# tpatten/squirrel_motion_planner

Hardware: AMD Instinct MI355X
Metric: collision-checked samples/sec + time-to-first-feasible-path, 8-DoF, 5 cm octomap (higher is better)
Workload: dtype f64

## Files before the change

### include/smp_gpu.h

```cpp
#ifndef SMP_GPU_H
#define SMP_GPU_H

#include <stddef.h>
#include <stdint.h>

#ifdef __cplusplus
extern "C" {
#endif

enum {
  SMP_OK = 0,
  SMP_ERR_ARG = -1,
  SMP_ERR_START_INVALID = -2,
  SMP_ERR_GOAL_INVALID = -3,
  SMP_ERR_NO_SOLUTION = -4,
  SMP_ERR_HIP = -5,
  SMP_ERR_PARSE = -6,
  SMP_ERR_CAPACITY = -7,
  SMP_ERR_NO_DEVICE = -8
};

enum { SMP_BUDGET_ITERATIONS = 0, SMP_BUDGET_SECONDS = 1, SMP_BUDGET_SAMPLES = 2 };

typedef struct smp_robot smp_robot;
typedef struct smp_scene smp_scene;
typedef struct smp_planner smp_planner;

typedef struct smp_scene_opts {
  double resolution;
  double z_offset;
  int insert_floor;
  double floor_center[2];
  double floor_distance;
} smp_scene_opts;

typedef struct smp_params {
  double near_threshold;
  double step_factor;
  int num_traj_segments;
  int max_near_nodes;
  double path_optimality_threshold;
  int tree_optimization;
  int informed_sampling;
  int64_t node_capacity;
  int helpers;
  int scout;
} smp_params;

typedef struct smp_query {
  double start[8];
  double goal[8];
  double env_x[2];
  double env_y[2];
  int check_self;
  int check_map;
  int budget_kind;
  double budget;
  uint64_t seed;
  uint32_t query_id;
} smp_query;

typedef struct smp_stats {
  int64_t iterations;
  int64_t first_solution_iter;
  int64_t last_solution_iter;
  int64_t configs_checked;
  int64_t configs_valid;
  double time_first_solution;
  double time_total;
  double cost_best[3];
  double cost_theoretical[3];
  int64_t nodes_start, nodes_goal, edges_start, edges_goal, rewires_start, rewires_goal;
  int32_t connected_tree_is_start;
  int32_t conn_node_b, conn_node_a;
  int64_t nn_nodes_scanned;
  int64_t near_nodes_scanned;
  int64_t samples_precomputed;
  double phase_seconds[32];
  int64_t scout_nn_hits;
  int64_t scout_near_hits;
  int64_t scout_edge_hits;
  int64_t scout_edge_misses;
  double scout_wait_seconds;
  double scout_phase_seconds[32];
  int32_t helpers;
  int32_t scout;
  double time_first_solution_host;
  int64_t scout_conn_row_hits;
  int64_t scout_conn_batch_hits;
  int64_t scout_conn_ov_hits;
} smp_stats;

typedef struct smp_result {
  int status;
  int64_t n_waypoints;
  double* waypoints;
  smp_stats stats;
  int64_t n_cost_rows;
  double* cost_rows;
} smp_result;

void smp_params_default(smp_params* p);
void smp_scene_opts_default(smp_scene_opts* o);

int smp_robot_create_json(const char* model_json, smp_robot** out);
int smp_robot_create_urdf(const char* urdf_xml, const char* srdf_xml, const char* spheres_json, smp_robot** out);
void smp_robot_destroy(smp_robot* r);
int smp_robot_num_links(const smp_robot* r);
const char* smp_robot_link_name(const smp_robot* r, int i);
int smp_robot_self_rounds(const smp_robot* r, int32_t info[8], uint16_t* sp_ab, double* sp_rr2, uint16_t* pp_ps,
                          int32_t* partner, double* rr2, uint32_t* prim_mask);

typedef struct smp_attach {
  const char* link;
  const char* name;
  int n_spheres;
  const double* centres;
  const double* radii;
  const char* const* touch_links; int n_touch;
} smp_attach;
int smp_robot_attach(const smp_robot* base, const smp_attach* a, smp_robot** out);
int smp_cover_box(const double half[3], const double pose[12], double tol, int max_spheres,
                  double* centres, double* radii, int* n);
int smp_cover_cylinder(double radius, double half_length, const double pose[12], double tol, int max_spheres,
                       double* centres, double* radii, int* n);

int smp_scene_from_keys(const uint16_t* keys_xyz, int64_t n, const smp_scene_opts* opts, smp_scene** out);
int smp_scene_from_bt(const uint8_t* data, size_t size, const smp_scene_opts* opts, smp_scene** out);
int smp_scene_from_ot(const uint8_t* data, size_t size, const smp_scene_opts* opts, smp_scene** out);
int smp_scene_from_octomap_msg(const char* id, double resolution, int binary, const uint8_t* data, size_t size,
                               const smp_scene_opts* opts, smp_scene** out);
int smp_scene_from_grid(const uint64_t* bits, const uint16_t* d2, const int dims[3], const double origin[3],
                        double resolution, smp_scene** out);
void smp_scene_destroy(smp_scene* s);
int smp_scene_info(const smp_scene* s, int dims[3], double origin[3], double* resolution,
                   int64_t* n_occupied, double bbox_min[3], double bbox_max[3]);
int smp_scene_export(const smp_scene* s, uint64_t* bits, uint16_t* d2);

int smp_planner_create(int device, const smp_robot* robot, const smp_params* params, smp_planner** out);
void smp_planner_destroy(smp_planner* p);
int smp_planner_set_scene(smp_planner* p, const smp_scene* s);
typedef struct smp_scene_build {
  int dims[3];
  double origin[3];
  double resolution;
  int64_t n_occupied;
  double bbox_min[3], bbox_max[3];
  double kernel_ms;
  double total_ms;
} smp_scene_build;
int smp_planner_set_scene_keys(smp_planner* p, const uint16_t* keys_xyz, int64_t n, const smp_scene_opts* opts,
                               smp_scene_build* info);
int smp_planner_set_scene_bt(smp_planner* p, const uint8_t* data, size_t size, const smp_scene_opts* opts,
                             smp_scene_build* info);
int smp_planner_set_scene_ot(smp_planner* p, const uint8_t* data, size_t size, const smp_scene_opts* opts,
                             smp_scene_build* info);
int smp_planner_set_scene_octomap_msg(smp_planner* p, const char* id, double resolution, int binary,
                                      const uint8_t* data, size_t size, const smp_scene_opts* opts,
                                      smp_scene_build* info);
typedef struct smp_carve {
  double q[8];
  double pad;
  const char* const* links; int n_links;
} smp_carve;
typedef struct smp_carve_info { int64_t n_carved; double kernel_ms, total_ms; } smp_carve_info;
int smp_planner_set_carve(smp_planner* p, const smp_carve* c);
int smp_planner_last_carve(const smp_planner* p, smp_carve_info* info);
int smp_carve_keys(smp_planner* p, const uint16_t* keys_xyz, int64_t n, const smp_scene_opts* opts,
                   const smp_carve* c, uint8_t* carved, smp_carve_info* info);
int smp_planner_set_params(smp_planner* p, const smp_params* params);
int smp_planner_get_params(const smp_planner* p, smp_params* params);
int smp_set_disabled_map_links(smp_planner* p, const char* const* link_names, int n);
int smp_planner_set_robot(smp_planner* p, const smp_robot* r);
// ... 183 lines not shown
```

### squirrel_motion_planner_amd/_lib.py

```python
import ctypes
import os

HERE = os.path.dirname(os.path.abspath(__file__))
LIB_PATH = os.environ.get("SMP_LIB") or os.path.join(HERE, "lib", "libsmp_gpu.so")
MODEL_JSON = os.path.join(HERE, "data", "robotino_model.json")
SPHERES_JSON = os.path.join(HERE, "data", "robotino_spheres.json")

SMP_OK = 0
SMP_ERR_ARG = -1
SMP_ERR_START_INVALID = -2
SMP_ERR_GOAL_INVALID = -3
SMP_ERR_NO_SOLUTION = -4
SMP_ERR_HIP = -5
SMP_ERR_PARSE = -6
SMP_ERR_CAPACITY = -7
SMP_ERR_NO_DEVICE = -8

BUDGET_ITERATIONS = 0
BUDGET_SECONDS = 1
BUDGET_SAMPLES = 2

_d = ctypes.c_double
_i = ctypes.c_int
_i64 = ctypes.c_int64
_p = ctypes.c_void_p
_pd = ctypes.POINTER(ctypes.c_double)


class SceneOpts(ctypes.Structure):
    _fields_ = [("resolution", _d), ("z_offset", _d), ("insert_floor", _i), ("floor_center", _d * 2),
                ("floor_distance", _d)]


class Params(ctypes.Structure):
    _fields_ = [("near_threshold", _d), ("step_factor", _d), ("num_traj_segments", _i), ("max_near_nodes", _i),
                ("path_optimality_threshold", _d), ("tree_optimization", _i), ("informed_sampling", _i),
                ("node_capacity", _i64), ("helpers", _i), ("scout", _i)]


class Query(ctypes.Structure):
    _fields_ = [("start", _d * 8), ("goal", _d * 8), ("env_x", _d * 2), ("env_y", _d * 2), ("check_self", _i),
                ("check_map", _i), ("budget_kind", _i), ("budget", _d), ("seed", ctypes.c_uint64),
                ("query_id", ctypes.c_uint32)]


class Stats(ctypes.Structure):
    _fields_ = [("iterations", _i64), ("first_solution_iter", _i64), ("last_solution_iter", _i64),
                ("configs_checked", _i64), ("configs_valid", _i64), ("time_first_solution", _d), ("time_total", _d),
                ("cost_best", _d * 3), ("cost_theoretical", _d * 3), ("nodes_start", _i64), ("nodes_goal", _i64),
                ("edges_start", _i64), ("edges_goal", _i64), ("rewires_start", _i64), ("rewires_goal", _i64),
                ("connected_tree_is_start", ctypes.c_int32), ("conn_node_b", ctypes.c_int32),
                ("conn_node_a", ctypes.c_int32), ("nn_nodes_scanned", _i64), ("near_nodes_scanned", _i64),
                ("samples_precomputed", _i64), ("phase_seconds", _d * 32), ("scout_nn_hits", _i64),
                ("scout_near_hits", _i64), ("scout_edge_hits", _i64), ("scout_edge_misses", _i64),
                ("scout_wait_seconds", _d), ("scout_phase_seconds", _d * 32), ("helpers", ctypes.c_int32),
                ("scout", ctypes.c_int32), ("time_first_solution_host", _d), ("scout_conn_row_hits", _i64),
                ("scout_conn_batch_hits", _i64), ("scout_conn_ov_hits", _i64)]


class Result(ctypes.Structure):
    _fields_ = [("status", _i), ("n_waypoints", _i64), ("waypoints", _pd), ("stats", Stats), ("n_cost_rows", _i64),
                ("cost_rows", _pd)]


class IkRequest(ctypes.Structure):
    _fields_ = [("ee_pose", _d * 6), ("deviation", (_d * 2) * 6), ("q_init", _d * 8), ("max_iter", _i)]


class IkResult(ctypes.Structure):
    _fields_ = [("reached", _i), ("iterations", _i), ("fallback_iterations", _i), ("q", _d * 8), ("error", _d * 6),
                ("manipulability", _d)]


class GoalSearch(ctypes.Structure):
    _fields_ = [("n_candidates", _i), ("n_reached", _i), ("chosen", _i), ("downward", _i), ("kernel_ms", _d)]


class SceneDevice(ctypes.Structure):
    _fields_ = [("dims", _i * 3), ("origin", _d * 3), ("resolution", _d), ("n_bricks", _i64), ("n_cells", _i64),
                ("n_prim", _i), ("has_d2b", _i), ("bricks", _p), ("d2", _p), ("d2b", _p), ("slab", _p)]


class SceneBuild(ctypes.Structure):
    _fields_ = [("dims", _i * 3), ("origin", _d * 3), ("resolution", _d), ("n_occupied", _i64), ("bbox_min", _d * 3),
                ("bbox_max", _d * 3), ("kernel_ms", _d), ("total_ms", _d)]


class Attach(ctypes.Structure):
    _fields_ = [("link", ctypes.c_char_p), ("name", ctypes.c_char_p), ("n_spheres", _i), ("centres", _pd),
                ("radii", _pd), ("touch_links", ctypes.POINTER(ctypes.c_char_p)), ("n_touch", _i)]


class Carve(ctypes.Structure):
    _fields_ = [("q", _d * 8), ("pad", _d), ("links", ctypes.POINTER(ctypes.c_char_p)), ("n_links", _i)]


class CarveInfo(ctypes.Structure):
    _fields_ = [("n_carved", _i64), ("kernel_ms", _d), ("total_ms", _d)]


class ShortcutInfo(ctypes.Structure):
    _fields_ = [("n_edges", _i64), ("n_valid", _i64), ("configs_checked", _i64), ("cost_in", _d), ("cost_out", _d),
                ("first_blocked", _i64), ("kernel_ms", _d), ("total_ms", _d)]


class Detour(ctypes.Structure):
    _fields_ = [("v", _d * 8), ("M1", ctypes.c_int32), ("M2", ctypes.c_int32), ("free", ctypes.c_int32),
                ("pad", ctypes.c_int32)]


class RepairOpts(ctypes.Structure):
    _fields_ = [("samples", _i), ("rounds", _i), ("seed", ctypes.c_uint64)]


class RepairInfo(ctypes.Structure):
    _fields_ = [("n_blocked_edges", _i64), ("n_gaps", _i64), ("n_repaired", _i64), ("n_items", _i64), ("n_free", _i64),
                ("rounds_used", ctypes.c_int32), ("cost_in", _d), ("cost_out", _d), ("first_blocked", _i64),
                ("kernel_ms", _d), ("total_ms", _d)]


class Margin(ctypes.Structure):
    _fields_ = [("map", _d), ("self", _d)]


class Clearance(ctypes.Structure):
    _fields_ = [("map", _d), ("self", _d), ("map_link", ctypes.c_int32), ("self_a", ctypes.c_int32),
                ("self_b", ctypes.c_int32), ("pad", ctypes.c_int32)]


class EdgeClearance(ctypes.Structure):
    _fields_ = [("map", _d), ("self", _d), ("map_point", ctypes.c_int32), ("self_point", ctypes.c_int32),
                ("map_link", ctypes.c_int32), ("self_a", ctypes.c_int32), ("self_b", ctypes.c_int32),
                ("n_points", ctypes.c_int32)]


class ClearanceInfo(ctypes.Structure):
    _fields_ = [("n_points", _i64), ("kernel_ms", _d), ("total_ms", _d)]


class BaseLattice(ctypes.Structure):
# ... 171 lines not shown
```

### squirrel_motion_planner_amd/csrc/smp_api_plan.cpp

```cpp
#include <hip/hip_runtime.h>

#include <algorithm>
#include <array>
#include <chrono>
#include <cmath>
#include <cstdio>
#include <cstdlib>
#include <cstring>
#include <thread>
#include <vector>

#include "smp_kernels.h"
#include "smp_planner.h"
#include "smp_provision.h"

using namespace smp;

static_assert(PROV_MAX_SCOUTS == MAX_SCOUTS && PROV_SCAN_P == SCAN_P && PROV_SCAN_PNEAR == SCAN_PNEAR,
              "smp_provision.h restates smp_plan.h");

static int resident_slots(smp_planner* p) {
  if (p->slots_cache > 0) return std::max(1, p->slots_cache / std::max(1, p->slot_share));
  int occ_plan = 0;
  if (hipOccupancyMaxActiveBlocksPerMultiprocessor(&occ_plan, reinterpret_cast<const void*>(&plan_kernel), BLOCK, 0) !=
// ... 435 lines not shown
    if (k.bounds) {
      int dbg[8];
      if (smp_debug_bounds(dbg) == 0 && dbg[0])
        std::fprintf(stderr, "[smp] bounds: %s:%d id %d block %d tree %d limit %d (launch %lld)\n", site_file(dbg[0]),
                     site_line(dbg[0]), dbg[1], dbg[2], dbg[3], dbg[4], (long long)c.launches);
    }
    float ms = 0;
    HIPCHK(hipEventElapsedTime(&ms, p->ev0, p->ev1));
    c.total_ms += ms;
    if (k.debug) {
      JobBoard jbh;
      const int i0 = act[0];
      if (nh > 0) HIPCHK(hipMemcpy(&jbh, c.qdev[i0].jb, sizeof(JobBoard), hipMemcpyDeviceToHost));
      std::fprintf(stderr, "[smp] launch %lld queries %d grid %d chunk %d: %.3f ms phase %d status %d iter %lld checked %lld"
                   " board stop %d job %u tile0 %llx\n", (long long)c.launches, na, na * (1 + nh), chunk, ms, S[i0].phase,
                   S[i0].status, S[i0].iter, S[i0].checked, nh ? jbh.stop : -1, nh ? (unsigned)(jbh.pay[0] >> 32) : 0u,
                   nh ? jbh.res[0] : 0ull);
    }
    std::vector<int> still;
    int solved_before = 0, solved_now = 0;
    for (int i : act) solved_before += sol_seen[i];
    for (int i : act)
      if (!(S[i].phase == 2 || S[i].status != 0)) still.push_back(i);
    for (int i : act) { sol_seen[i] = S[i].have_sol ? 1 : 0; solved_now += sol_seen[i]; }
    const bool shrank = still.size() < act.size();
    act.swap(still);
    if (act.empty()) break;
    if (shrank || (ns > c.prov.ns_base && solved_now != solved_before)) {
      if (k.rebalance) provision_queries(c, act);
      if (int st = upload_active(c)) return st;
    }
    if (chunk < 4096) chunk *= 2;
  }
  hstamp(c, "launch loop done");
#ifdef SMP_RING_CHECK
  smp_ringchk_dump();
#endif
  return SMP_OK;
}

static int plan_assemble(PlanCall& c, smp_result* out, std::vector<char>& done) {
  smp_planner* p = c.p;
  const int nq = c.nq;
  QState* S = c.S;
  HIPCHK(hipMemcpyAsync(p->d_qdev.p, c.qdev.data(), nq * sizeof(QueryDev), hipMemcpyHostToDevice, p->stream));
  p->last_plan_ms = c.total_ms;
  p->last_plan_launches = c.launches;

  hipLaunchKernelGGL(path_kernel, dim3(nq), dim3(64), 0, p->stream, p->d_qdev.p, p->d_counts.p);
  HIPCHK(hipGetLastError());
  std::vector<int> counts(2 * nq);
  HIPCHK(hipMemcpyAsync(counts.data(), p->d_counts.p, 2 * nq * sizeof(int), hipMemcpyDeviceToHost, p->stream));
  HIPCHK(hipStreamSynchronize(p->stream));
  int rc = SMP_OK;
  for (int i = 0; i < nq; ++i) {
    QState& s = S[i];
    smp_result& r = out[i];
    r.status = s.status != 0 ? s.status : (s.have_sol ? SMP_OK : SMP_ERR_NO_SOLUTION);
    smp_stats& st = r.stats;
    st.iterations = s.iter;
    st.first_solution_iter = s.first_iter;
    st.last_solution_iter = s.last_iter;
    st.configs_checked = s.checked;
    st.configs_valid = s.valid;
    st.time_first_solution = s.have_sol && s.t_first >= s.t0 ? (double)(s.t_first - s.t0) / p->wall_rate_hz : -1.0;
    st.time_total = s.t_end >= s.t0 ? (double)(s.t_end - s.t0) / p->wall_rate_hz : 0.0;
    st.time_first_solution_host = s.have_sol ? c.host_ttff[i] : -1.0;
    for (int k = 0; k < 3; ++k) { st.cost_best[k] = s.cbest[k]; st.cost_theoretical[k] = s.h0[k]; }
    st.nodes_start = s.n[0]; st.nodes_goal = s.n[1];
    st.edges_start = s.edges[0]; st.edges_goal = s.edges[1];
    st.rewires_start = s.rewires[0]; st.rewires_goal = s.rewires[1];
    st.connected_tree_is_start = s.conn_start;
    st.conn_node_b = s.nB.id; st.conn_node_a = s.nA.id;
    st.nn_nodes_scanned = s.nn_nodes;
    st.near_nodes_scanned = s.near_nodes;
    st.samples_precomputed = s.smp_hits;
    st.scout_nn_hits = s.sc_nn;
    st.scout_near_hits = s.sc_near;
    st.scout_edge_hits = s.sc_edge_hit;
    st.scout_edge_misses = s.sc_edge_miss;
    st.scout_conn_row_hits = s.sc_conn_row;
    st.scout_conn_batch_hits = s.sc_conn_batch;
    st.scout_conn_ov_hits = (int64_t)c.scout_conn_ov[i];
    st.scout_wait_seconds = (double)s.sc_wait / p->wall_rate_hz;
    for (int k = 0; k < 32; ++k) {
      const bool count = k == 8 || k == 11 || (k >= 20 && k < 28) || k == 30;
      st.scout_phase_seconds[k] = count ? (double)c.scout_prof[i][k] : (double)c.scout_prof[i][k] / p->wall_rate_hz;
    }
    st.helpers = c.nh_first;
    st.scout = c.ns_first;
    for (int k = 0; k < 32; ++k)
      st.phase_seconds[k] = (k == 8 || k == 11 || k >= 20) ? (double)s.prof[k] : (double)s.prof[k] / p->wall_rate_hz;
    if (i == 0) { p->last_n[0] = s.n[0]; p->last_n[1] = s.n[1]; }
    r.n_cost_rows = s.n_rows;
    if (s.n_rows > 0) {
      r.cost_rows = (double*)malloc(sizeof(double) * 5 * s.n_rows);
      HIPCHK(hipMemcpy(r.cost_rows, p->qb[i].rows.p, sizeof(double) * 5 * s.n_rows, hipMemcpyDeviceToHost));
      for (int64_t k = 0; k < s.n_rows; ++k) r.cost_rows[k * 5 + 1] /= p->wall_rate_hz;
    }
    if (r.status != SMP_OK) { done[i] = 1; continue; }
    const int n_sp = counts[2 * i], n_gp = counts[2 * i + 1];
    const int np = p->params.num_traj_segments;
    std::vector<double> pe((size_t)(n_sp + n_gp) * 2 * NJ);
    if (n_sp + n_gp > 0) {
      HIPCHK(p->d_path_edges.reserve(pe.size()));
      const int nthr = (int)pe.size();
      hipLaunchKernelGGL(path_edges_kernel, dim3((nthr + 255) / 256), dim3(256), 0, p->stream, p->d_qdev.p, i, n_sp,
                         n_gp, p->d_path_edges.p);
      HIPCHK(hipGetLastError());
      HIPCHK(hipMemcpyAsync(pe.data(), p->d_path_edges.p, pe.size() * sizeof(double), hipMemcpyDeviceToHost, p->stream));
      HIPCHK(hipStreamSynchronize(p->stream));
    }
    std::vector<double> wp;
    for (int k = 0; k < n_sp + n_gp; ++k) {
      const double* a = &pe[(size_t)k * 2 * NJ];
      const double* b = a + NJ;
      double stp[NJ];
      for (int j = 0; j < NJ; ++j) stp[j] = (b[j] - a[j]) / double(np);
      if (k < n_sp) {
        for (int inc = 0; inc < np; ++inc)
          for (int j = 0; j < NJ; ++j) wp.push_back(a[j] + inc * stp[j]);
      } else {
        for (int inc = np; inc > 0; --inc)
          for (int j = 0; j < NJ; ++j) wp.push_back(a[j] + inc * stp[j]);
        if (k == n_sp + n_gp - 1)
          for (int j = 0; j < NJ; ++j) wp.push_back(a[j] + 0 * stp[j]);
      }
    }
    r.n_waypoints = (int64_t)(wp.size() / NJ);
    if (!wp.empty()) {
      r.waypoints = (double*)malloc(sizeof(double) * wp.size());
      std::memcpy(r.waypoints, wp.data(), sizeof(double) * wp.size());
    }
    done[i] = 1;
  }
  for (int i = 0; i < nq; ++i) if (out[i].status != SMP_OK && rc == SMP_OK) rc = out[i].status;
  hstamp(c, "results assembled");
  return rc;
}

static int plan_batch_impl(smp_planner* p, const smp_query* qs, int nq, smp_result* out, std::vector<char>& done) {
  PlanCall c;
  c.t_entry = std::chrono::steady_clock::now();
  c.p = p;
  c.qs = qs;
  c.nq = nq;
  c.k = read_plan_knobs(p->params.helpers, nq);
  if (int st = plan_prepare(c)) return st;
  if (int st = plan_launch_loop(c)) return st;
  return plan_assemble(c, out, done);
}

extern "C" int smp_plan_batch(smp_planner* p, const smp_query* qs, int nq, smp_result* out) {
  if (!p || !qs || nq <= 0 || !out) return SMP_ERR_ARG;
  for (int i = 0; i < nq; ++i) std::memset(&out[i], 0, sizeof(smp_result));
  if (int b_ = busy_check(p)) {
    for (int i = 0; i < nq; ++i) out[i].status = b_;
    return b_;
  }
  std::vector<char> done(nq, 0);
  const int rc = plan_batch_impl(p, qs, nq, out, done);
  if (rc == SMP_ERR_HIP) (void)hipGetLastError();
  for (int i = 0; i < nq; ++i) {
    if (done[i]) continue;
    smp_result_free(&out[i]);
    out[i].status = rc != SMP_OK ? rc : SMP_ERR_HIP;
// ... 73 lines not shown
```

### squirrel_motion_planner_amd/csrc/smp_kernels.hip

```cpp
#include <hip/hip_runtime.h>

#include <vector>

#include "smp_collide.h"
#include "smp_kernels.h"
#include "smp_math.h"
#include "smp_plan.h"
#include "smp_types.h"

extern "C" __device__ __attribute__((const)) unsigned long long __ockl_wfred_min_u64(unsigned long long);
extern "C" __device__ __attribute__((const)) unsigned long long __ockl_wfred_max_u64(unsigned long long);

namespace smp {

constexpr int CHECK_CT = 32;

__shared__ RobotDev g_rb;
__shared__ MapCfg g_mc;
__shared__ WideStash g_wk;

template <int CT>
__global__ void __launch_bounds__(BLOCK) check_kernel_t(const RobotDev* __restrict__ rb, SceneDev sc,
                                                        const MapCfg* __restrict__ mc, const double* __restrict__ q,
                                                        long long n, int self, int map, uint8_t* __restrict__ valid,
// ... 271 lines not shown
static_assert(sizeof(ViaNode) == 8 * (3 * NJ + 3 + 1), "ViaNode as 8-byte words: q, c, e_start, e_target, {id, parent}");
static_assert(VIA_B * VIA_WORDS <= BLOCK, "one ViaNode word per thread");
struct PlanLds {
  QState S;
  union {
    struct {
      TileLds<PLAN_CT> T;
      double tq[PLAN_CT][NJ];
    } tile;
    JobLds job;
    double seg[MAXE][MAX_PTS][3];
    ViaLds via;
    SmpLds smp;
    SamplerLds smpl;
  } u;
  union {
    struct {
      struct {
        unsigned long long wlk[BLOCK / 64][MAX_NEAR], whk[BLOCK / 64][MAX_NEAR];
        int wli[BLOCK / 64][MAX_NEAR], whi[BLOCK / 64][MAX_NEAR];
        int wtot[BLOCK / 64];
      } nr;
      struct {
        alignas(16) unsigned hist[NEAR_BINS];
        unsigned long long ck[2][NEAR_BUF];
        int ci[2][NEAR_BUF];
        unsigned long long wmin[BLOCK / 64], wmax[BLOCK / 64];
        int wtot[BLOCK / 64];
        int cnt[2], blo, bhi, fast;
      } nh;
    };
    struct {
      ScanLds s;
      MergeLds m;
    } sc;
  };
  double eg_start[MAXE][NJ], eg_target[MAXE][NJ], eg_step[MAXE][NJ], eg_end[MAXE][NJ];
  double eg_base[MAXE][3], eg_cost[MAXE][3];
  double eg_acc[MAXE][3];
  int eg_first[MAXE], eg_need[MAXE], eg_near[MAXE], eg_ptr[MAXE];
  int eg_par[MAXE];
  int conn_need0;
  int rw_par[MAXE], rw_next;
  double rw_cost[MAXE][3];
  int tile_e[PLAN_CT], tile_i[PLAN_CT], tile_n;
  int count_slot;
  int job_seq;
  int in_job;
  int go_end;
  int smp_ver, smp_have_sol, smp_hit;
  int smp_pub;
  int spec, spec_nn;
  long long spec_cnt;
  double smp_cbest[3];
  int nk;
  unsigned long long near_blo, near_bhi;
  int lo_i[MAX_NEAR], hi_i[MAX_NEAR];
  double lo_c[MAX_NEAR], hi_c[MAX_NEAR];
  int n_lo, n_hi;
  NodeRef nn, xn, xc, cur, g;
  double xr[NJ], ext[NJ], ox[NJ];
  double en_start[NJ], en_target[NJ];
  int ext_nn, ext_bp, flag, found, nn_id, cnt;
  int reached;
  int n_via, nn_t, tree_expand;
  NodeRef sel;
  double sel_start[NJ], sel_target[NJ];
  double csp[3], best_nv;
  double sol[3];
  double wd[BLOCK / 64];
  unsigned long long wk[BLOCK / 64];
  int wi[BLOCK / 64];
  long long wcount[BLOCK / 64];
  ScoutRec sr;
  PreRec prer;
  int prer_ok;
#ifdef SMP_TRACE
  int trole;
  unsigned tn;
  long long tit;
  int tbar;
#endif
  int sp_on, sp_stage, sp_go[2];
  double fnn_d;
  int fnn_id;
#ifdef SMP_SCAN_PROF
  unsigned long long spc_t;
#endif
  int sc_same[MAX_SCOUTS];
  unsigned sc_seen, sc_dead;
  int asked[SCOUT_SLOTS];
  int asked_conn[SCOUT_SLOTS];
  int asked_pre[SCOUT_SLOTS];
  int two_scouts;
  unsigned sc_mod;
  unsigned rw_at0;
  int n_at0;
  int sc_t, sc_rerun;
  int sc_stale_f;
  int ov_local, conn_ov;
  unsigned conn_ov_n;
#ifdef SMP_CONN_PROF
  unsigned cprof[12];
#endif
  double sc_hq[MAXE][NJ], sc_hc[MAXE];
  int sc_hp[MAXE];
  int rb_go[2];
  long long sc_k;
  int eg_hit[MAXE];
  int eg_rec[MAXE];
  int rec_grp;
  int rec_all, ev_job;
  double pc_q[2][PATCH_K][NJ];
};

__shared__ PlanLds g_L;
static_assert(sizeof(ViaLds) <= sizeof(g_L.u.seg), "a via chain's batch lies within the union's edge rows");

struct Ctx {
  SceneDev sc;
  QueryDev Q;
};

}
#include "smp_plan_prof.h"
namespace smp {

__device__ __forceinline__ int lane_id() { return threadIdx.x & 63; }
__device__ __forceinline__ int uni(int v) { return __builtin_amdgcn_readfirstlane(v); }
__device__ __forceinline__ int wave_id() { return threadIdx.x >> 6; }
typedef const double __attribute__((address_space(1)))* gcdptr;
__device__ __forceinline__ gcdptr uni_gptr(const double* p) {
  const unsigned long long v = reinterpret_cast<unsigned long long>(p);
  const unsigned lo = __builtin_amdgcn_readfirstlane((int)(unsigned)v);
  const unsigned hi = __builtin_amdgcn_readfirstlane((int)(unsigned)(v >> 32));
  return (gcdptr)(((unsigned long long)hi << 32) | lo);
}

__device__ __forceinline__ gcdptr uni_g(gcdptr p) {
  const unsigned long long v = reinterpret_cast<unsigned long long>(p);
  const unsigned lo = __builtin_amdgcn_readfirstlane((int)(unsigned)v);
  const unsigned hi = __builtin_amdgcn_readfirstlane((int)(unsigned)(v >> 32));
  return (gcdptr)(((unsigned long long)hi << 32) | lo);
}
__device__ __forceinline__ void tree_cols(gcdptr tq, int cap, gcdptr* c) {
#pragma unroll
  for (int j = 0; j < NJ; ++j) c[j] = uni_g(tq + (size_t)j * (unsigned)cap);
}
__device__ __forceinline__ bool wave_group_live(int first, int end) {
  return __builtin_amdgcn_readfirstlane((int)(first < end)) != 0;
}
__device__ __forceinline__ double ld_col(gcdptr col, unsigned i) {
  return *(gcdptr)((const char __attribute__((address_space(1)))*)col + i * 8u);
}
typedef const float __attribute__((address_space(1)))* gcfptr;
__device__ __forceinline__ float ld_col(gcfptr col, unsigned i) {
  return *(gcfptr)((const char __attribute__((address_space(1)))*)col + i * 4u);
}
template <int K, int NPT, typename P, typename T>
__device__ __forceinline__ void load_round_k(T (*a)[NJ], const P* cols, int b0, int i1, const T* fill) {
#pragma unroll
  for (int u = 0; u < NPT; ++u) {
    if (u < K) {
      const unsigned ii = (unsigned)min(b0 + u * BLOCK, i1 - 1);
#pragma unroll
      for (int j = 0; j < NJ; ++j) a[u][j] = ld_col(cols[j], ii);
    } else {
#pragma unroll
      for (int j = 0; j < NJ; ++j) a[u][j] = fill[j];
    }
  }
}
template <int NPT, typename P, typename T>
__device__ __forceinline__ void load_round(T (*a)[NJ], const P* cols, int b0, int i1, const T* fill) {
  static_assert(NPT == 8, "rounds of 8 nodes per thread");
  const int first = b0 - lane_id();
  const int nl = uni(min(NPT, (i1 - first + BLOCK - 1) / BLOCK));
  if (nl > 4) load_round_k<8, NPT>(a, cols, b0, i1, fill);
  else if (nl > 2) load_round_k<4, NPT>(a, cols, b0, i1, fill);
  else if (nl > 1) load_round_k<2, NPT>(a, cols, b0, i1, fill);
  else load_round_k<1, NPT>(a, cols, b0, i1, fill);
}

__device__ __forceinline__ void st_tree(double* p, double v) { *p = v; }
__device__ __forceinline__ void st_tree(int* p, int v) { *p = v; }
__device__ __forceinline__ void st_tree(float* p, float v) { *p = v; }
__device__ __forceinline__ void st_coord(const TreeDev& T, int cap, int j, int i, double v) {
  st_tree(&T.q[(size_t)j * cap + i], v);
  st_tree(&T.qf[(size_t)j * cap + i], (float)v);
}
__device__ __forceinline__ int xcc_id() { return __builtin_amdgcn_s_getreg((3 << 11) | 20); }
__device__ __forceinline__ bool same8(const double* a, const double* b) {
  bool s = true;
#pragma unroll
  for (int j = 0; j < NJ; ++j) s &= __double_as_longlong(a[j]) == __double_as_longlong(b[j]);
  return s;
}

#define load_node(C, t, id, o) load_node_at(C, t, id, o, SMP_SITE)
__device__ __forceinline__ void load_node_at(const Ctx& C, int t, int id, NodeRef* o, int site) {
  const TreeDev& T = C.Q.tr[t];
  const int cap = g_L.S.cap;
  BCHK(id, cap, site, t);
  (void)site;
  for (int j = 0; j < NJ; ++j) o->q[j] = T.q[(size_t)j * cap + id];
  for (int k = 0; k < 3; ++k) o->c[k] = T.cost[(size_t)k * cap + id];
  o->id = id;
  o->parent = T.parent[id];
}

__device__ void insert_node(const Ctx& C, int t, const double* e_start, const double* e_target, const NodeRef& x) {
  QState& S = g_L.S;
  int i = S.n[t];
  if (i >= S.cap || x.id != i) { S.status = -7; S.phase = 2; return; }
  const TreeDev& T = C.Q.tr[t];
  int cap = S.cap;
  for (int j = 0; j < NJ; ++j) {
    st_coord(T, cap, j, i, x.q[j]);
    T.e_start[(size_t)j * cap + i] = e_start[j];
    T.e_target[(size_t)j * cap + i] = e_target[j];
    g_L.pc_q[t][i & (PATCH_K - 1)][j] = x.q[j];
  }
  for (int k = 0; k < 3; ++k) st_tree(&T.cost[(size_t)k * cap + i], x.c[k]);
  st_tree(&T.parent[i], x.parent);
  T.first_child[i] = -1;
  int p = x.parent;
  int f = T.first_child[p];
  T.next_sib[i] = f;
  T.prev_sib[i] = -1;
  if (f >= 0) T.prev_sib[f] = i;
  T.first_child[p] = i;
  S.n[t] = i + 1;
  S.edges[t]++;
}

__device__ bool spec_stage(const Ctx& C, int s, unsigned long long wait = 0);
__device__ __forceinline__ int scan_parts(const Ctx& C, int near, int nodes) {
  int P = min(min(C.Q.nworkers, SCAN_P), near ? min(min(C.Q.scan_pnear, SCAN_PNEAR), max(8, nodes >> C.Q.scan_nshift)) : C.Q.scan_pnn);
  if (g_L.in_job) P = min(P, max(C.Q.nworkers - g_L.u.job.ntiles, 8));
  return uni(P);
}
__device__ __forceinline__ bool scan_split(const Ctx& C, int nodes) {
  return uni(C.Q.jb != nullptr && C.Q.scan_min > 0 && nodes >= C.Q.scan_min && C.Q.nworkers >= 8 && !g_L.ov_local);
}
__device__ int nearest_dist(const Ctx& C, int t, const double* q, int i0, int n, double* d_out);
__device__ void near_set_dist(const Ctx& C, int t, const double* q, int excl, bool nn);
constexpr int LOCAL_F32_MIN = 2048;
struct ScanLds;
__device__ __forceinline__ void slice_nn_body32(gcdptr tq, const float* tqf, int cap, int i0, int i1, const double* q,
                                                ScanLds& X);
__device__ __forceinline__ int nearest_scan(const Ctx& C, int t, const double* q, int i_begin, double* d_out) {
  TR();
  if (scan_split(C, uni(g_L.S.n[t]) - i_begin)) {
    int id;
    [[clang::always_inline]] id = nearest_dist(C, t, q, i_begin, uni(g_L.S.n[t]), d_out);
    return id;
  }
  const gcdptr tq = uni_gptr(C.Q.tr[t].q);
  const int n = uni(g_L.S.n[t]), cap = uni(g_L.S.cap);
  if (n - i_begin >= LOCAL_F32_MIN) {
    slice_nn_body32(tq, C.Q.tr[t].qf, cap, i_begin, n, q, g_L.sc.s);
    *d_out = __longlong_as_double((long long)g_L.sc.s.wk[0]);
    const int id = g_L.sc.s.wi[0];
    __syncthreads();
    return id;
  }
  gcdptr tqc[NJ];
  tree_cols(tq, cap, tqc);
  double qq[NJ];
  for (int j = 0; j < NJ; ++j) qq[j] = q[j];
  double best = 10000.0, best_s = 1e300;
  int bid = 0x7fffffff;
  constexpr int NPT = 8;
  for (int i0 = i_begin + threadIdx.x; i0 < n; i0 += NPT * BLOCK) {
    double a[NPT][NJ];
    load_round<NPT>(a, tqc, i0, n, qq);
    double s[NPT];
#pragma unroll
    for (int u = 0; u < NPT; ++u) s[u] = 0.0;
#pragma unroll
    for (int j = 0; j < NJ; ++j) {
#pragma unroll
      for (int u = 0; u < NPT; ++u) {
        const double d = qq[j] - a[u][j];
        s[u] += d * d;
      }
    }
#pragma unroll
    for (int u = 0; u < NPT; ++u) {
      const int i = i0 + u * BLOCK;
      if (i < n && s[u] < best_s) {
        const double dist = sqrt(s[u]);
        if (dist < best) { best = dist; bid = i; best_s = s[u]; }
      }
    }
  }
  TR();
  const unsigned long long key = (unsigned long long)__double_as_longlong(best);
  const unsigned long long wk = __ockl_wfred_min_u64(key);
  const int wi = __ockl_wfred_min_i32(key == wk ? bid : 0x7fffffff);
  if (lane_id() == 0) { g_L.wk[wave_id()] = wk; g_L.wi[wave_id()] = wi; }
  __syncthreads();
  unsigned long long bk = g_L.wk[0];
  int bi = g_L.wi[0];
#pragma unroll
  for (int w = 1; w < BLOCK / 64; ++w) {
    const unsigned long long k = g_L.wk[w];
    const int i = g_L.wi[w];
    if (k < bk || (k == bk && i < bi)) { bk = k; bi = i; }
  }
  __syncthreads();
  *d_out = __longlong_as_double((long long)bk);
  TR();
  return bi;
}

__device__ int patch_scan(int t, const double* q, int i0, int n, double* d_out) {
  if (threadIdx.x < 64) {
    const int i = i0 + (int)threadIdx.x;
// ... 1416 lines not shown
    }
    const unsigned long long lb = __ballot(live);
    if (lane == 0) J.tskip = lb == 0;
  }
  __syncthreads();
  return uni(J.tskip) != 0;
}

struct DirectJob {
  unsigned hdr;
  int ne;
};
__device__ __forceinline__ unsigned job_tile_mask(const Ctx& C, const WideConst& K, JobLds& J, int t,
                                                  unsigned long long* prof = nullptr, int seq = -1,
                                                  const DirectJob* direct = nullptr, bool sync_after = true) {
  int ct, nc, self, map;
  bool sk = false;
  if (direct) {
    const unsigned hdr = direct->hdr;
    const int ne = direct->ne;
    const int np1 = (int)((hdr >> 8) & 255);
    ct = 1 << ((hdr >> 21) & 3);
    const int base = t * ct;
    nc = min(ct, ne * np1 - base);
    self = (int)((hdr >> 16) & 1);
    map = (int)((hdr >> 17) & 1);
    const int c = (int)(threadIdx.x >> 6) / (NWAVE / ct), j = threadIdx.x & 63;
    if (c < nc && j < NJ) {
      const int sl = base + c, k = sl / np1, i = sl - k * np1, wi = 1 + 32 * k + 2 * j;
      const double qs = __hiloint2double((int)J.words[wi + 1], (int)J.words[wi]);
      const double qd = __hiloint2double((int)J.words[wi + 2 * NJ + 1], (int)J.words[wi + 2 * NJ]);
      J.tq[c][j] = qs + i * qd;
    }
    wave_sync();
  } else {
    ct = uni(J.ct);
    const int base = t * ct;
    nc = min(ct, uni(J.nslots) - base);
    self = J.self;
    map = J.map;
    sk = seq >= 0 && uni(J.skip) && t >= uni(C.Q.nworkers);
    if (sk && job_tile_skip(C, J, t, seq)) return 0u;
    if (threadIdx.x < nc * NJ) {
      const int c = threadIdx.x / NJ, j = threadIdx.x - c * NJ;
      const int sl = base + c, k = sl / J.np1, i = sl - k * J.np1;
      J.tq[c][j] = J.start[k][j] + i * J.step[k][j];
    }
    if (threadIdx.x < TILE_CT_MAX) J.T.coll[threadIdx.x] = 0;
    __syncthreads();
  }
  const TileOrder order{J.tgrp, J.tord, J.first, false};
  collide_wide((&g_rb), K, ct, nc, J.tq, self, map, J.T, sk ? &order : nullptr, prof);
  unsigned m = 0;
  for (int c = 0; c < nc; ++c) m |= (J.T.coll[c] ? 1u : 0u) << c;
  if (sync_after) __syncthreads();
  return m;
}

__device__ __noinline__ unsigned job_tile_mask_out(const Ctx& C, JobLds& J, int t, int seq) {
  const WideConst K = wide_const_load(g_wk, C.sc);
  return job_tile_mask(C, K, J, t, nullptr, seq);
}

enum { OV_NONE = 0, OV_NEAR_EXPAND = 1, OV_NN = 2, OV_NEAR_XN = 3 };
__device__ void overlap_work(const Ctx& C, int ov, int t);
__device__ void conn_window(const Ctx& C, int t);
__device__ __forceinline__ bool take_spec(int ov) {
  const bool hit = uni(g_L.spec) == ov;
  __syncthreads();
  if (hit && threadIdx.x == 0) {
    (ov == OV_NN ? g_L.S.nn_nodes : g_L.S.near_nodes) += g_L.spec_cnt;
    g_L.spec = OV_NONE;
  }
  __syncthreads();
  return hit;
}

enum { EARLY_NONE = 0, EARLY_EXPAND = 1, EARLY_CHOOSE = 2, EARLY_REWIRE = 3 };
constexpr int EDGE_EARLY_W = (int)(offsetof(ScoutEdge, first) / 8);
static_assert(EDGE_EARLY_W == 2 * NJ + 3, "ScoutEdge: s, g, acc, then {first, pad}");
__device__ __forceinline__ int sc_stale_now(const ScoutBoard* sb) {
  return (long long)ld_agent(&sb->cur) > g_L.sc_k || ld_agent(&sb->stop);
}
__device__ __forceinline__ void sc_early_send(const Ctx& C, int early, int epar, int E, bool read_stale) {
  if (early == EARLY_NONE) return;
  ScoutBoard* sb = C.Q.scb;
  ScoutRec* rec = &sb->rec[epar];
  if (read_stale && threadIdx.x == 0) g_L.sc_stale_f = sc_stale_now(sb);
  const int g0 = early == EARLY_EXPAND ? 0 : early == EARLY_CHOOSE ? SCOUT_CHOOSE0 : SCOUT_REWIRE0;
  for (int i = threadIdx.x; i < E * EDGE_EARLY_W; i += BLOCK) {
    const int e = i / EDGE_EARLY_W, k = i - e * EDGE_EARLY_W;
    const double v = k < NJ ? g_L.eg_start[e][k] : k < 2 * NJ ? g_L.eg_target[e][k - NJ] : g_L.eg_acc[e][k - 2 * NJ];
    st_agent(reinterpret_cast<unsigned long long*>(&rec->e[g0 + e]) + k, (unsigned long long)__double_as_longlong(v));
  }
  if (early == EARLY_EXPAND) {
    constexpr int XW = (int)(sizeof(ScoutExpand) / 8);
    static_assert(XW == 3 * NJ + 3 + 1 && offsetof(ScoutExpand, ok) == (XW - 1) * 8, "ScoutExpand: ext, step, end, acc, {ok, pad}");
    const int k = (int)threadIdx.x - 64;
    if (k >= 0 && k < XW) {
      unsigned long long w;
      if (k == XW - 1) w = *reinterpret_cast<const unsigned long long*>(&g_L.sr.ex.ok);
      else w = (unsigned long long)__double_as_longlong(k < NJ ? g_L.eg_target[0][k] : k < 2 * NJ ? g_L.eg_step[0][k - NJ] :
                                                        k < 3 * NJ ? g_L.eg_end[0][k - 2 * NJ] : g_L.eg_acc[0][k - 3 * NJ]);
      st_agent(reinterpret_cast<unsigned long long*>(&rec->ex) + k, w);
    }
  } else {
    const int k = (int)threadIdx.x - (BLOCK - 64);
    if (k >= 0 && k < 2) st_agent(reinterpret_cast<unsigned long long*>(&rec->n_choose) + k,
                                  reinterpret_cast<const unsigned long long*>(&g_L.sr.n_choose)[k]);
  }
}
__device__ __forceinline__ void sc_first_send(const Ctx& C, int early, int epar, int E) {
  const int g0 = early == EARLY_EXPAND ? 0 : early == EARLY_CHOOSE ? SCOUT_CHOOSE0 : SCOUT_REWIRE0;
  if ((int)threadIdx.x < E) {
    const int e = threadIdx.x;
    const int first = g_L.eg_need[e] ? g_L.eg_first[e] : -1;
    st_agent(reinterpret_cast<unsigned long long*>(&C.Q.scb->rec[epar].e[g0 + e]) + EDGE_EARLY_W,
             (unsigned long long)(unsigned)first);
  }
}

__device__ __forceinline__ void job_header(const Ctx& C, bool need, bool sfv) {
  auto& J = g_L.u.job;
  const int e = threadIdx.x;
  const int np1 = g_L.S.n_pts + 1;
  const int W = max(1, C.Q.nworkers);
  const unsigned long long m = __ballot(need);
  const int k = __popcll(m & ((1ull << e) - 1));
  if (need) J.emap[k] = e;
  if (e == 0) {
    const int ne = __popcll(m);
    J.E = ne;
    J.np1 = np1;
    J.nslots = ne * np1;
    J.ct = job_tile_ct(ne * np1, W, C.Q.tile_ct);
    J.ntiles = (ne * np1 + J.ct - 1) / J.ct;
    J.self = g_L.S.self; J.map = g_L.S.map;
    J.seq = ++g_L.job_seq;
    J.skip = J.ntiles > W;
    J.sfv = J.skip && sfv;
  }
}
__device__ __forceinline__ void edge_validity_job(const Ctx& C, int E, int pslot, int ov, int ovt, int early = 0,
                                                  int epar = 0, bool conn_b = false) {
  JobBoard* jb = C.Q.jb;
  auto& J = g_L.u.job;
  const int np1 = g_L.S.n_pts + 1;
  const int W = max(1, C.Q.nworkers);
  const int ne = uni(J.E), nt = uni(J.ntiles), seq = uni(J.seq), ct = uni(J.ct);
  const unsigned long long tj0 = threadIdx.x == 0 ? wall_clock64() : 0;
  for (int i = threadIdx.x; i < 1 + 32 * ne; i += BLOCK) {
    unsigned w;
    if (i == 0) {
      w = (unsigned)ne | (unsigned)np1 << 8 | (unsigned)(J.self != 0) << 16 | (unsigned)(J.map != 0) << 17 |
          (unsigned)J.skip << 19 | (unsigned)J.sfv << 20 | (unsigned)__builtin_ctz((unsigned)J.ct) << 21;
    } else {
      const int m = i - 1, k = m >> 5, r = m & 31, j = (r & 15) >> 1, e = J.emap[k];
      const unsigned long long bits = (unsigned long long)__double_as_longlong(r < 16 ? g_L.eg_start[e][j] : g_L.eg_step[e][j]);
      w = (r & 1) ? (unsigned)(bits >> 32) : (unsigned)bits;
    }
    st_agent(&jb->pay[i], granule(seq, w));
  }
  for (int it = threadIdx.x; it < ne * NJ; it += BLOCK) {
    const int k = it / NJ, j = it - k * NJ, e = J.emap[k];
    J.start[k][j] = g_L.eg_start[e][j];
    J.step[k][j] = g_L.eg_step[e][j];
  }
  for (int t = threadIdx.x; t < nt; t += BLOCK) J.rdone[t] = 0;
  if (threadIdx.x < ne) J.first[threadIdx.x] = np1;
  JOBPROF_PUBLISHED(jb);
  PROF_BEGIN();
  if (threadIdx.x == 0) { g_L.S.prof[P_TFK] += _pt - tj0; g_L.S.prof[P_TTEST]++; }
  TR();
  if (threadIdx.x == 0) g_L.in_job = 1;
  sc_early_send(C, early, epar, E, false);
  __syncthreads();
  if (conn_b) conn_window(C, ovt);
  else overlap_work(C, ov, ovt);
  if (threadIdx.x == 0) g_L.in_job = 0;
  TR();
  const bool skip = uni(J.skip) != 0;
  for (int t = W - 1; t < nt; t += W) {
    const unsigned m = job_tile_mask_out(C, J, t, skip ? seq : -1);
    if (threadIdx.x == 0) {
      J.rmask[t] = m;
      J.rdone[t] = 1;
      if (skip) st_agent(&jb->res[t], granule(seq, m));
    }
  }
  __syncthreads();
  const unsigned long long tj1 = threadIdx.x == 0 ? wall_clock64() : 0;
  if (threadIdx.x == 0) g_L.S.prof[P_TCHAIN] += tj1 - _pt;
  unsigned long long t_prog = tj1, t_wait = tj1;
  int last_left = 1 << 30;
  for (int k = 0;; k ^= 1) {
    if (threadIdx.x < 64) {
      int left = 0;
      unsigned long long cur_v = 0;
      int stop_v = 0;
      if (early != EARLY_NONE && threadIdx.x == 0) { cur_v = ld_agent(&C.Q.scb->cur); stop_v = ld_agent(&C.Q.scb->stop); }
      for (int t = threadIdx.x; t < nt; t += 64) {
// ... 447 lines not shown
      }
      if (go > 0 && threadIdx.x < TILE_CT_MAX) J.T.coll[threadIdx.x] = 0;
      if (threadIdx.x == 0) {
        if (go == 0 && (ld_agent(&jb->stop) || wall_clock64() - t_last > 200000000ull)) go = -1;
        J.go[k] = go;
        J.seq = go == -3 ? (int)stag : (int)tag0;
      }
    }
    __syncthreads();
    const int go = uni(J.go[k]);
    if (go == -1) break;
    if (go == 0) {
      __builtin_amdgcn_s_sleep(SMP_HELPER_SLEEP);
      continue;
    }
    const int seq = uni(J.seq);
    if (go == -3) {
      scan_helper(C, J, w, seq);
      last_scan = seq;
      t_last = wall_clock64();
      continue;
    }
    const unsigned hdr = J.words[0];
    const int ne = min((int)(hdr & 255), MAXE), nw = 1 + 32 * ne;
    if (go == -2) {
      int bad = 0;
      for (int i = PU * 64 + threadIdx.x; i < nw; i += BLOCK) {
        const unsigned long long v = ld_agent(&jb->pay[i]);
        if ((int)(v >> 32) != seq) bad = 1;
        J.words[i] = (unsigned)v;
      }
      if (threadIdx.x == 0) J.left = 0;
      __syncthreads();
      if (bad) J.left = 1;
      __syncthreads();
      if (uni(J.left)) continue;
    }
    auto decode = [&]() {
      for (int it = threadIdx.x; it < ne * 2 * NJ; it += BLOCK) {
        const int kk = it / (2 * NJ), r = it - kk * 2 * NJ;
        const int wi = 1 + 32 * kk + 2 * r;
        const double d = __hiloint2double((int)J.words[wi + 1], (int)J.words[wi]);
        if (r < NJ) J.start[kk][r] = d; else J.step[kk][r - NJ] = d;
      }
      if (threadIdx.x == 0) {
        J.E = ne;
        J.np1 = (int)((hdr >> 8) & 255);
        J.self = (hdr >> 16) & 1;
        J.map = (hdr >> 17) & 1;
        J.skip = (hdr >> 19) & 1;
        J.sfv = (hdr >> 20) & 1;
        J.nslots = ne * J.np1;
        J.ct = 1 << ((hdr >> 21) & 3);
        J.ntiles = (J.nslots + J.ct - 1) / J.ct;
      }
      if (hdr & (1u << 19))
        for (int t = threadIdx.x; t < JOB_TILES; t += BLOCK) J.rdone[t] = 0;
    };
    JOBPROF_TILE_CLOCKS(J, tp);
    const int nt = (ne * (int)((hdr >> 8) & 255) + (1 << ((hdr >> 21) & 3)) - 1) >> ((hdr >> 21) & 3);
    const bool direct = go > 0;
    last = seq;
    JOBPROF_PICKUP(jb, w, nt);
    if (w - 1 >= nt) __syncthreads();
    bool decoded = false;
    const DirectJob dj{hdr, ne};
    for (int t = w - 1; t < nt; t += W) {
      const bool dt = direct && t == w - 1;
      if (!dt && !decoded) {
        decode();
        __syncthreads();
        decoded = true;
      }
      const unsigned m = job_tile_mask(C, K, J, t, tp, seq, dt ? &dj : nullptr, false);
      if (threadIdx.x == 0) st_agent(&jb->res[t], granule(seq, m));
      __syncthreads();
      JOBPROF_TILE_DONE(jb);
    }
    JOBPROF_TILES_OUT(jb, J, w, nt);
    t_last = wall_clock64();
  }
}

__device__ __forceinline__ void sc_copy_out(ScoutBoard* sb, int par, const void* p, int nbytes) {
  const size_t off = (const char*)p - (const char*)&g_L.sr;
  const unsigned long long* src = (const unsigned long long*)p;
  unsigned long long* dst = (unsigned long long*)((char*)&sb->rec[par] + off);
  for (int w = threadIdx.x; w < nbytes / 8; w += BLOCK) st_agent(&dst[w], src[w]);
}
__device__ __forceinline__ void sc_copy_in(const ScoutBoard* sb, int par, void* p, int nbytes) {
  const size_t off = (const char*)p - (const char*)&g_L.sr;
  unsigned long long* dst = (unsigned long long*)p;
  const unsigned long long* src = (const unsigned long long*)((const char*)&sb->rec[par] + off);
  for (int w = threadIdx.x; w < nbytes / 8; w += BLOCK) dst[w] = ld_agent(&src[w]);
}
static_assert(sizeof(ScoutNN) % 8 == 0 && sizeof(ScoutNear) % 8 == 0 && sizeof(ScoutEdge) % 8 == 0 &&
              sizeof(ScoutExpand) % 8 == 0 && offsetof(ScoutRec, ex) % 8 == 0 && offsetof(ScoutRec, nr) % 8 == 0 &&
              sizeof(ScoutConnect) % 8 == 0 && offsetof(ScoutRec, cn) % 8 == 0 && sizeof(ScoutConn) % 8 == 0 &&
              sizeof(ScoutPre) % 8 == 0 && offsetof(ScoutRec, pre) % 8 == 0 && sizeof(ViaNode) % 8 == 0 &&
              offsetof(ScoutRec, cc) % 8 == 0 && offsetof(ScoutRec, n_choose) % 8 == 0 && offsetof(ScoutRec, e) % 8 == 0,
              "scout record sections are 8-byte words");

constexpr unsigned long long SCOUT_WAIT = 6000;
#ifndef SMP_CONN_WAIT
#define SMP_CONN_WAIT 2000
#endif

__device__ void spec_copy(const ScoutBoard* sb, int par, int have, int st);
__device__ bool spec_stage(const Ctx& C, int s, unsigned long long wait) {
  if (!uni(g_L.sp_on)) return false;
  if (wait == 0) wait = SCOUT_WAIT;
  const int have = uni(g_L.sp_stage);
  if (have >= s) return true;
  const ScoutBoard* sb = C.Q.scbs[uni(g_L.asked[g_L.S.iter & (SCOUT_SLOTS - 1)]) - 1];
  const int par = (int)(g_L.S.iter & (SCOUT_SLOTS - 1));
  const unsigned tag = (unsigned)(g_L.S.iter + 1);
  const unsigned long long t0 = threadIdx.x == 0 ? wall_clock64() : 0;
  TR();
  int got;
  for (int k = 0;; k ^= 1) {
    if (threadIdx.x == 0) {
      const unsigned long long v = ld_agent(&sb->stage[par]);
      const unsigned lo = (unsigned)v;
      const bool cur = ((lo >> 8) & 0xfffu) == (g_L.rw_at0 & 0xfffu);
      int go = 0;
      if ((unsigned)(v >> 32) != tag) go = -1;
      else if (cur && (int)(lo & 0xffu) >= s) go = 1 + (int)(lo & 0xffu);
      else if (wall_clock64() - t0 > wait) go = -1;
      g_L.sp_go[k] = go;
    }
    __syncthreads();
    got = uni(g_L.sp_go[k]);
    if (got != 0) break;
    __builtin_amdgcn_s_sleep(1);
  }
  if (threadIdx.x == 0) g_L.S.sc_wait += wall_clock64() - t0;
  WAIT_CLOCK(s, t0);
  TR();
  if (got < 0) {
    if (threadIdx.x == 0) g_L.sp_on = 0;
    __syncthreads();
    return false;
  }
  spec_copy(sb, par, have, got - 1);
  TR();
  return true;
}

__device__ void spec_copy(const ScoutBoard* sb, int par, int have, int st) {
  ScoutRec& R = g_L.sr;
  const bool opt_now = uni(g_L.S.tree_opt && g_L.S.have_sol) != 0;
  int off[8], nw[8], ns = 0;
  auto add = [&](const void* p, int nbytes) {
    off[ns] = (int)((const char*)p - (const char*)&R) / 8;
    nw[ns] = nbytes / 8;
    ++ns;
  };
  if (have < SC_NN && st >= SC_NN) add(&R.nn, sizeof(ScoutNN));
  if (have < SC_EXPAND && st >= SC_EXPAND) { add(&R.e[0], sizeof(ScoutEdge)); add(&R.ex, sizeof(ScoutExpand)); }
  if (have < SC_NEAR && st >= SC_NEAR) add(&R.nr, sizeof(ScoutNear));
  if ((have < SC_CHOOSE && st >= SC_CHOOSE) || (have < SC_DONE && st >= SC_DONE)) add(&R.n_choose, 4 * sizeof(int));
  if (opt_now && have < SC_CHOOSE && st >= SC_CHOOSE) add(&R.e[SCOUT_CHOOSE0], MAX_NEAR * sizeof(ScoutEdge));
  if (opt_now && have < SC_DONE && st >= SC_DONE) add(&R.e[SCOUT_REWIRE0], MAX_NEAR * sizeof(ScoutEdge));
  if (!opt_now && have < SC_DONE && st >= SC_DONE) { add(&R.cn, sizeof(ScoutConnect)); add(&R.pre, sizeof(ScoutPre)); }
  if (have < SC_CONN && st >= SC_CONN) add(&R.cc, sizeof(ScoutConn));
  int total = 0;
  for (int i = 0; i < ns; ++i) total += nw[i];
  const unsigned long long* src = reinterpret_cast<const unsigned long long*>(&sb->rec[par]);
  unsigned long long* dst = reinterpret_cast<unsigned long long*>(&R);
  constexpr int U = 4;
  static_assert(sizeof(ScoutRec) / 8 <= U * BLOCK, "one round per record copy");
  int idx[U];
  unsigned long long v[U];
#pragma unroll
  for (int u = 0; u < U; ++u) {
    const int w = (int)threadIdx.x + u * BLOCK;
    idx[u] = -1;
    if (w < total) {
      int rem = w, i = 0;
      while (rem >= nw[i]) { rem -= nw[i]; ++i; }
      idx[u] = off[i] + rem;
      v[u] = ld_agent(&src[idx[u]]);
    }
  }
#pragma unroll
  for (int u = 0; u < U; ++u)
    if (idx[u] >= 0) dst[idx[u]] = v[u];
  __syncthreads();
  if (threadIdx.x == 0) g_L.sp_stage = st;
  __syncthreads();
}

__device__ void scout_ask(const Ctx& C, long long k, int tree, bool pre, bool& fenced, int x_snap = -1) {
  const QState& S = g_L.S;
  const int ns = C.Q.nscouts;
  int which = 1 + (int)(pre ? (unsigned)k % (unsigned)ns : (ns >= 2 ? (unsigned)(k & 1) : 0u));
  if ((g_L.sc_dead >> (which - 1)) & 1u) {
    if (!pre) return;
    int w = -1;
    for (int d = 1; d < ns && w < 0; ++d) {
      const int c = (int)((unsigned)(k + d) % (unsigned)ns);
      if (!((g_L.sc_dead >> c) & 1u)) w = c;
    }
    if (w < 0) return;
    for (int x = 0; x < SCOUT_SLOTS; ++x)
      if (g_L.asked[x] == 1 + w) return;
    which = 1 + w;
  }
  ScoutBoard* sb = C.Q.scbs[which - 1];
  int& same = g_L.sc_same[which - 1];
  if (same < 0) {
    const int x = ld_agent(&sb->xcc);
    if (x > 0) same = (x - 1) == xcc_id() ? 1 : 0;
  }
  if (same != 1 && !fenced) {
    __builtin_amdgcn_fence(__ATOMIC_RELEASE, "agent");
    drain();
    fenced = true;
  }
  const unsigned tag = (unsigned)(k + 1);
  const unsigned w0 = (unsigned)(x_snap >= 0 ? x_snap : S.n[tree]) | (unsigned)tree << 28 | (unsigned)(!pre) << 29;
  st_agent(&sb->req[2], granule(tag, (unsigned)S.n[1 - tree]));
  st_agent(&sb->req[1], granule(tag, ((unsigned)g_L.smp_ver & 0xfffffu) | ((unsigned)S.rewires[tree] & 0xfffu) << 20));
  st_agent(&sb->req[0], granule(tag, w0));
  g_L.asked[k & (SCOUT_SLOTS - 1)] = which;
  g_L.asked_conn[k & (SCOUT_SLOTS - 1)] = !pre && ns >= 2;
  g_L.asked_pre[k & (SCOUT_SLOTS - 1)] = pre;
}

__device__ void scout_ask_early(const Ctx& C, int stage_j) {
  const QState& S = g_L.S;
  if (!C.Q.early_ask || C.Q.nscouts < 2 || !(S.tree_opt && S.have_sol) || stage_j < SC_DONE) return;
  const long long k = S.iter + 2;
  if (g_L.asked[k & (SCOUT_SLOTS - 1)]) return;
  const int w = (int)(k & 1);
  if (g_L.sc_same[w] != 1 || ((g_L.sc_dead >> w) & 1u)) return;
  bool fenced = true;
  scout_ask(C, k, S.A, false, fenced, g_L.n_at0);
}

__device__ void scout_slots() {
  const QState& S = g_L.S;
  const long long j = S.iter;
  g_L.rw_at0 = (unsigned)S.rewires[S.A];
  g_L.n_at0 = S.n[S.A];
  g_L.asked[(j - 1) & (SCOUT_SLOTS - 1)] = 0;
  g_L.asked_conn[(j - 1) & (SCOUT_SLOTS - 1)] = 0;
  g_L.sp_on = g_L.asked[j & (SCOUT_SLOTS - 1)] != 0 &&
              !(g_L.asked_pre[j & (SCOUT_SLOTS - 1)] && S.have_sol && j >= S.first_iter + 3);
  g_L.sp_stage = -1;
}
__device__ __forceinline__ void scout_cur_lanes(const Ctx& C) {
  const QState& S = g_L.S;
  const long long j = S.iter;
  const int s = (int)lane_id();
  if (s >= C.Q.nscouts) return;
  const bool pre = !(S.tree_opt && S.have_sol);
  const int nsc = pre ? C.Q.nscouts : min(C.Q.nscouts, 2);
  ScoutBoard* sb = C.Q.scbs[s];
  if (!pre && j == S.first_iter + 3 && s >= 2) st_agent(&sb->stop, 1);
  if (s >= nsc) return;
  st_agent(&sb->cur, (unsigned long long)j);
  if (pre && S.n[0] < (1 << 20) && S.n[1] < (1 << 20) && g_L.sc_same[s] == 1)
    st_agent(&sb->cur_sz, ((unsigned long long)(j & 0xffffff) << 40) | ((unsigned long long)S.n[0] << 20) |
                              (unsigned long long)S.n[1]);
}
__device__ void scout_asks(const Ctx& C, int t) {
  const QState& S = g_L.S;
  const long long j = S.iter;
  const bool pre = !(S.tree_opt && S.have_sol);
  bool fenced = false;
  for (int ahead = 1; ahead <= (pre ? C.Q.nscouts : 1); ++ahead) {
    const long long k = j + ahead;
// ... 650 lines not shown
      for (int i = 0; i < 2; ++i) {
        double s = 0.0;
        for (int k = 0; k < 2; ++k) s += (S.Cpr[i * 2 + k] * lp[k]) * bp[k];
        rp[i] = s + S.ctr_pr[i];
      }
      {
        int cr = 0, cp = 0;
#pragma unroll
        for (int j = 0; j < NJ; ++j) {
          const bool rv = rb->rev[j] != 0;
          double v = 0.0;
#pragma unroll
          for (int i = 0; i < 6; ++i) v = rv && cr == i ? rr[i] : v;
#pragma unroll
          for (int i = 0; i < 2; ++i) v = !rv && cp == i ? rp[i] : v;
          r[j] = v;
          cr += rv ? 1 : 0;
          cp += rv ? 0 : 1;
        }
      }
      bool above = 0.0 <= ee_z(rb, r);
      bool inside = (r[0] < S.env_x[1] && r[0] > S.env_x[0] && r[1] < S.env_y[1] && r[1] > S.env_y[0]) || env0;
      unsigned long long m = __ballot(above && inside && lane < SE_OUT);
      const int w = m ? __ffsll((long long)m) - 1 : -1;
      if (lane == w) for (int j = 0; j < NJ; ++j) out[j] = r[j];
      if (lane == 0) W.win = w;
    }
    __syncthreads();
    if (uni(W.win) >= 0) return 0;
  }
}

__device__ __forceinline__ int sample_conf(const QState& S, uint32_t it, SmpLds& W, double* out) {
  if (uni(S.informed && S.have_sol)) return sample_ellipse(S, it, W, out);
  return sample_uniform(S, it, W, out);
}

__device__ void sample_version(const Ctx& C) {
  QState& S = g_L.S;
  g_L.smp_pub = 0;
  if (!C.Q.sampler) return;
  const bool changed = g_L.smp_ver == 0 || g_L.smp_have_sol != S.have_sol || g_L.smp_cbest[0] != S.cbest[0] ||
                       g_L.smp_cbest[1] != S.cbest[1] || g_L.smp_cbest[2] != S.cbest[2];
  if (changed) {
    g_L.smp_have_sol = S.have_sol;
    for (int k = 0; k < 3; ++k) g_L.smp_cbest[k] = S.cbest[k];
    ++g_L.smp_ver;
    g_L.smp_pub = 1;
  }
}
__device__ void sample_publish(const Ctx& C, bool before_read = false) {
  if (!C.Q.sampler) return;
  const QState& S = g_L.S;
  JobBoard* jb = C.Q.jb;
  if (g_L.smp_pub) {
    st_agent(&jb->s_have_sol, g_L.smp_have_sol);
    for (int k = 0; k < 3; ++k) st_agent(&jb->s_cbest[k], (unsigned long long)__double_as_longlong(g_L.smp_cbest[k]));
    drain();
    st_agent(&jb->s_ver, g_L.smp_ver);
  }
  st_agent(reinterpret_cast<unsigned long long*>(&jb->s_iter), (unsigned long long)(S.iter - (before_read ? 1 : 0)));
}

__device__ __forceinline__ bool pre_read_round(const ScoutBoard* sb, int par, unsigned tag) {
  const int g = (int)threadIdx.x - 64;
  if (g < 0 || g >= PRE_GRANULES) return true;
  const unsigned long long v = ld_agent(&sb->pre_g[par][g]);
  reinterpret_cast<unsigned*>(&g_L.prer)[g] = (unsigned)v;
  return (unsigned)(v >> 32) == tag;
}

__device__ __forceinline__ void sample_read(const Ctx& C) {
  TR();
  QState& S = g_L.S;
  const uint32_t it = (uint32_t)S.iter;
  const bool pre = uni(g_L.sp_on && g_L.sp_stage < 0) != 0;
  const int sw = uni(g_L.asked[S.iter & (SCOUT_SLOTS - 1)]);
  const ScoutBoard* sb = sw > 0 ? C.Q.scbs[sw - 1] : nullptr;
  const int par = (int)(S.iter & (SCOUT_SLOTS - 1));
  const bool prerec = pre && !uni(S.have_sol);
  bool pre_ok = true;
  if (prerec) pre_ok = pre_read_round(sb, par, (unsigned)(S.iter + 1));
  if (threadIdx.x == 64) {
    int st = -1;
    if (pre && !prerec) {
      const unsigned long long v = ld_agent(&sb->stage[par]);
      const unsigned lo = (unsigned)v;
      if ((unsigned)(v >> 32) == (unsigned)(S.iter + 1) && ((lo >> 8) & 0xfffu) == (g_L.rw_at0 & 0xfffu))
        st = (int)(lo & 0xffu);
    }
    g_L.sp_go[0] = st;
  }
  if (C.Q.sampler && threadIdx.x < 64) {
    JobBoard* jb = C.Q.jb;
    const unsigned want = ring_tag(it, (unsigned)__builtin_amdgcn_readfirstlane(g_L.smp_ver));
    unsigned long long v = 0;
    if (threadIdx.x < RING_G) v = ld_agent(&jb->ring[it % SMP_RING].g[threadIdx.x]);
    const int pk = (int)threadIdx.x - 2 * NJ;
    const bool ok = threadIdx.x >= RING_G ||
                    ((unsigned)(v >> 32) == want && (pk < 0 || (unsigned)v == ring_param(pk, S.have_sol, S.cbest)));
    const unsigned hi = (unsigned)odd_lane_of_pair((int)(unsigned)v);
    if (threadIdx.x < 2 * NJ && !(threadIdx.x & 1))
      g_L.xr[threadIdx.x >> 1] = __longlong_as_double((long long)(((unsigned long long)hi << 32) | (unsigned)v));
    const bool all = __ballot(!ok) == 0;
    if (threadIdx.x == 0) { g_L.smp_hit = all; if (all) S.smp_hits++; }
  } else if (threadIdx.x == 0) {
    g_L.smp_hit = 0;
  }
  drain();
  const bool stale_granule = __syncthreads_or(!pre_ok) != 0;
  TR();
  const bool prer_ok = prerec && !stale_granule;
  if (threadIdx.x < 64) {
    if (threadIdx.x == 0) {
      g_L.prer_ok = prer_ok;
      if (prer_ok) g_L.sc_seen |= 1u << (sw - 1);
      sample_publish(C);
    }
    TR();
    if (C.Q.nscouts > 0) scout_cur_lanes(C);
    TR();
  } else if (threadIdx.x == 64 && C.Q.nscouts > 0) {
    scout_asks(C, 1 - g_L.S.A);
    scout_ask_early(C, g_L.sp_go[0]);
  }
  TR();
  const int st = uni(g_L.sp_go[0]);
  __syncthreads();
  if (pre && !prerec && st >= 0) spec_copy(sb, par, -1, st);
  if (prer_ok && !uni(g_L.smp_hit) && uni(g_L.prer.t >= 0)) {
    if (threadIdx.x < NJ) g_L.xr[threadIdx.x] = g_L.prer.xr[threadIdx.x];
    if (threadIdx.x == 0) g_L.smp_hit = 1;
    __syncthreads();
  }
  if (!uni(g_L.smp_hit)) {
    if (sample_conf(S, it, g_L.u.smp, g_L.xr) < 0 && threadIdx.x == 0) { S.status = -1; S.phase = 2; }
    __syncthreads();
  }
  else ring_check_sample(S, it);
}

__device__ void cost_update(const Ctx& C, int t, int v, const double* red) {
  QState& S = g_L.S;
  const TreeDev& T = C.Q.tr[t];
  const int cap = S.cap;
  int* stack = C.Q.stack;
  int sp = 0;
  stack[sp++] = v;
  const bool connected = (t == 0) == (S.conn_start != 0);
  int visits = 0;
  while (sp > 0) {
    if (++visits > S.n[t]) { S.status = -7; S.phase = 2; return; }
    int id = stack[--sp];
    BCHK(id, cap, __LINE__, t);
    double nc[3];
    for (int k = 0; k < 3; ++k) { nc[k] = T.cost[(size_t)k * cap + id] + red[k]; st_tree(&T.cost[(size_t)k * cap + id], nc[k]); }
    if (S.have_sol) {
      if (id == S.nB.id && connected) {
        for (int k = 0; k < 3; ++k) { S.cbest[k] = S.cbest[k] + red[k]; S.nB.c[k] = nc[k]; }
        S.last_iter = S.iter;
      }
      if (id == S.nA.id && !connected) {
        for (int k = 0; k < 3; ++k) { S.cbest[k] = S.cbest[k] + red[k]; S.nA.c[k] = nc[k]; }
        S.last_iter = S.iter;
      }
    }
    for (int c = T.first_child[id]; c >= 0; c = T.next_sib[c]) {
      if (sp >= cap) { S.status = -7; S.phase = 2; return; }
      stack[sp++] = c;
    }
  }
}

__device__ __forceinline__ int choose_prefix() {
  const int lane = lane_id();
  const int m = g_L.nk > 0 ? min(g_L.n_lo, g_L.S.max_near) : 0;
  const bool below = lane < m && g_L.lo_c[lane] < g_L.xn.c[0];
  return min(m, (int)__builtin_ctzll(~__ballot(below)));
}
__device__ __forceinline__ void cur_from_batch(int e) {
  for (int j = 0; j < NJ; ++j) g_L.cur.q[j] = g_L.eg_start[e][j];
  for (int k = 0; k < 3; ++k) g_L.cur.c[k] = g_L.eg_base[e][k];
  g_L.cur.id = g_L.eg_near[e];
  g_L.cur.parent = g_L.eg_par[e];
}
__device__ void choose_parent(const Ctx& C, int t) {
  if (threadIdx.x < 64) {
    const int E = choose_prefix();
    if (threadIdx.x == 0) {
      g_L.ext_bp = 0;
      g_L.found = -1;
      g_L.cnt = E;
      if (g_L.nk > 0) g_L.xn.parent = g_L.nn.id;
    }
  }
  __syncthreads();
  TR();
  const int E = uni(g_L.cnt);
  if (E > 0) {
    if (threadIdx.x < E) {
      int e = threadIdx.x;
      NodeRef nd;
      load_node(C, t, g_L.lo_i[e], &nd);
      for (int j = 0; j < NJ; ++j) { g_L.eg_start[e][j] = nd.q[j]; g_L.eg_target[e][j] = g_L.xn.q[j]; }
      for (int k = 0; k < 3; ++k) g_L.eg_base[e][k] = nd.c[k];
      g_L.eg_near[e] = nd.id;
      g_L.eg_par[e] = nd.parent;
    }
    __syncthreads();
    TR();
    if (C.Q.jb && rec_match(C, E, SC_CHOOSE)) edge_costs_rec(E);
    else edge_costs(C, E);
// ... 697 lines not shown
      near_set_scan<20, false>(C, A, g_L.xn.q, g_L.xn.id);
    TR();
    PHASE(P_NEAR);
    choose_parent(C, A);
    TR();
    PHASE(P_CHOOSE);
  }
  if (uni(g_L.ext_nn || g_L.ext_bp)) {
    TR();
    if (threadIdx.x == 0) {
      insert_node(C, A, g_L.en_start, g_L.en_target, g_L.xn);
      g_L.spec = OV_NONE;
    }
    __syncthreads();
    TR();
    if (opt) {
      rewire(C, A);
      TR();
      scout_request_ahead2(C, A);
    }
    TR();
    PHASE(P_REWIRE);
    int cid;
    const bool crec = opt && conn_stage(C, B);
    TR();
    if (take_spec(OV_NN)) {
      cid = uni(g_L.spec_nn);
    } else if (crec) {
      cid = uni(g_L.sr.cc.d < 10000.0 ? g_L.sr.cc.id : 0);
      if (threadIdx.x == 0) { g_L.S.nn_nodes += g_L.S.n[B]; g_L.S.sc_nn++; }
    } else if (uni(!opt && g_L.sp_on) && spec_stage(C, SC_DONE, 2500) &&
               uni(g_L.sr.cn.ok && g_L.sr.cn.t == B &&
                   g_L.sr.cn.X <= g_L.S.n[B] && same8(g_L.sr.cn.q, g_L.xn.q))) {
      const int n = uni(g_L.S.n[B]);
      double dp = 10000.0;
      int ip = 0;
      if (uni(g_L.sr.cn.X < n)) ip = nearest_scan(C, B, g_L.xn.q, g_L.sr.cn.X, &dp);
      if (threadIdx.x == 0) { g_L.S.nn_nodes += n; g_L.S.sc_nn++; }
      cid = uni(dp < g_L.sr.cn.d ? ip : (g_L.sr.cn.d < 10000.0 ? g_L.sr.cn.id : 0));
    } else {
      cid = nearest(C, B, g_L.xn.q);
    }
    TR();
    const bool xrow = crec && uni(g_L.sr.cc.nrow >= 0) && cid == uni(g_L.sr.cc.d < 10000.0 ? g_L.sr.cc.id : 0);
    if (!xrow) {
      if (threadIdx.x == 0) load_node(C, B, cid, &g_L.xc);
      __syncthreads();
    }
    TR();
    PHASE(P_NN);
    connect_graphs(C, B, crec, xrow);
    TR();
    PHASE(P_CONNECT);
  }
  else if (opt) {
    scout_request_ahead2(C, A);
  }
  }
#undef PHASE
  if (threadIdx.x == 0) {
    QState& S = g_L.S;
    S.A = B;
    S.iter++;
    if (C.Q.rows && S.n_rows < C.Q.rows_cap) {
      double* row = C.Q.rows + S.n_rows * 5;
      row[0] = (double)S.iter;
      row[1] = (double)(wall_clock64() - S.t0);
      row[2] = S.cbest[0]; row[3] = S.cbest[1]; row[4] = S.cbest[2];
      S.n_rows++;
    }
    if ((S.cbest[0] - S.h0[0]) < S.opt_thresh) S.phase = 2;
    if (S.iter >= S.max_iter) S.phase = 2;
    if (S.max_checked && S.checked >= S.max_checked) S.phase = 2;
    if (S.has_deadline && wall_clock64() >= S.deadline) S.phase = 2;
    if (S.stop_margin && (S.n[0] + S.stop_margin > S.cap || S.n[1] + S.stop_margin > S.cap)) {
      S.phase = 2;
      if (!S.have_sol) S.status = -7;
    }
  }
  __syncthreads();
  TR_BARRIERS();
}

__device__ void sc_publish(const Ctx& C, int par, unsigned tag, int stage) {
  const unsigned long long t0 = threadIdx.x == 0 ? wall_clock64() : 0;
  drain();
  __syncthreads();
  if (threadIdx.x == 0) {
    st_agent(&C.Q.scb->stage[par], granule(tag, (unsigned)stage | (g_L.sc_mod & 0xfffu) << 8));
    g_L.S.prof[P_SC_PUBLISH] += wall_clock64() - t0;
  }
  __syncthreads();
}
#define SC_PHASE(k) if (threadIdx.x == 0) { const unsigned long long _t = wall_clock64(); g_L.S.prof[k] += _t - _ts; _ts = _t; }
__device__ bool sc_stale(const Ctx& C, unsigned tag) {
  if (threadIdx.x == 0) g_L.sp_go[0] = (long long)ld_agent(&C.Q.scb->cur) > (long long)tag - 1 || ld_agent(&C.Q.scb->stop);
  __syncthreads();
  const int s = uni(g_L.sp_go[0]);
  __syncthreads();
  return s != 0;
}

__device__ bool sc_moved(const Ctx& C) {
  if (!C.Q.early_ask) return false;
  if (threadIdx.x == 0)
    g_L.sc_rerun = (ld_agent(&C.Q.scb->rwb[g_L.sc_t]) & 0xfffu) != g_L.sc_mod &&
                   (long long)ld_agent(&C.Q.scb->cur) < g_L.sc_k;
  __syncthreads();
  const int r = uni(g_L.sc_rerun);
  __syncthreads();
  return r != 0;
}

__device__ void scout_connect(const Ctx& C, long long it, int t, int par, unsigned tag) {
  ScoutRec& R = g_L.sr;
  ScoutBoard* sb = C.Q.scb;
  const int tb = 1 - t;
  const bool scanned = uni(g_L.conn_ov) != 0;
  CONNPROF_CLOCK(_c0);
  for (int k = 0; !scanned; k ^= 1) {
    if (threadIdx.x == 0) {
      const unsigned long long v = ld_agent(&sb->cgo);
      int go = 0;
      if ((unsigned)(v >> 32) == tag) { go = 1; g_L.cnt = (int)(unsigned)v; }
      else if ((long long)ld_agent(&sb->cur) > it || ld_agent(&sb->stop)) go = -1;
      g_L.sp_go[k] = go;
    }
    __syncthreads();
    const int go = uni(g_L.sp_go[k]);
    if (go < 0) {
      __syncthreads();
      return;
    }
    if (go > 0) break;
    __builtin_amdgcn_s_sleep(2);
  }
  CONNPROF_CLOCK(_c1);
  if (!scanned) {
    __builtin_amdgcn_fence(__ATOMIC_ACQUIRE, "agent");
    if (threadIdx.x == 0) g_L.S.n[tb] = g_L.cnt;
    __syncthreads();
    [[clang::always_inline]] near_set<20, true>(C, tb, g_L.xn.q, g_L.xn.id);
  }
  CONNPROF_CLOCK(_c2);
  if (threadIdx.x == 0) {
    double d = g_L.fnn_d;
    int cid = g_L.fnn_id;
    if (!(d < 10000.0)) { cid = 0; d = 10000.0; }
    R.cc.d = d; R.cc.id = cid;
    load_node(C, tb, cid, &g_L.xc);
  }
  __syncthreads();
  if (threadIdx.x == 0) {
    const int E = min(g_L.n_lo, g_L.S.max_near);
    g_L.cnt = E;
    for (int j = 0; j < NJ; ++j) { g_L.eg_start[0][j] = g_L.xc.q[j]; g_L.eg_target[0][j] = g_L.xn.q[j]; }
    for (int k = 0; k < 3; ++k) g_L.eg_base[0][k] = 0.0;
  }
  __syncthreads();
  const int E = uni(g_L.cnt);
  if (threadIdx.x < E) {
    const int e = threadIdx.x;
    NodeRef nd;
    load_node(C, tb, g_L.lo_i[e], &nd);
    for (int j = 0; j < NJ; ++j) { g_L.eg_start[1 + e][j] = nd.q[j]; g_L.eg_target[1 + e][j] = g_L.xn.q[j]; }
    for (int k = 0; k < 3; ++k) g_L.eg_base[1 + e][k] = 0.0;
    if (e < CONN_ROWS) {
      for (int j = 0; j < NJ; ++j) R.cc.rq[e][j] = nd.q[j];
      for (int k = 0; k < 3; ++k) R.cc.rcost[e][k] = nd.c[k];
      R.cc.rparent[e] = nd.parent;
    }
  }
  __syncthreads();
  edge_costs(C, 1 + E);
  if (uni(C.Q.conn_check)) {
    if (threadIdx.x < MAXE) g_L.eg_need[threadIdx.x] = threadIdx.x < 1 + E;
    if (threadIdx.x == 0) g_L.rec_grp = -1;
    __syncthreads();
    [[clang::always_inline]] edge_validity(C, 1 + E, false, P_XCONNECT);
    if (threadIdx.x < E) R.cc.first[threadIdx.x] = g_L.eg_first[1 + threadIdx.x];
    if (threadIdx.x == 0) { R.cc.first0 = g_L.eg_first[0]; R.cc.nfirst = E; }
  }
  if (threadIdx.x < MAX_NEAR) {
    R.cc.lo_i[threadIdx.x] = g_L.lo_i[threadIdx.x]; R.cc.lo_c[threadIdx.x] = g_L.lo_c[threadIdx.x];
    R.cc.hi_i[threadIdx.x] = g_L.hi_i[threadIdx.x]; R.cc.hi_c[threadIdx.x] = g_L.hi_c[threadIdx.x];
  }
  if (threadIdx.x < E * 3) {
    const int e = threadIdx.x / 3, k = threadIdx.x - e * 3;
    R.cc.acc[e][k] = g_L.eg_acc[1 + e][k];
  }
  if (threadIdx.x == 0) {
    for (int j = 0; j < NJ; ++j) R.cc.q[j] = g_L.xn.q[j];
    for (int k = 0; k < 3; ++k) R.cc.acc0[k] = g_L.eg_acc[0][k];
    R.cc.X = g_L.S.n[tb]; R.cc.t = tb; R.cc.excl = g_L.xn.id;
    R.cc.nk = g_L.nk; R.cc.n_lo = g_L.n_lo; R.cc.n_hi = g_L.n_hi;
    for (int j = 0; j < NJ; ++j) R.cc.xq[j] = g_L.xc.q[j];
    for (int k = 0; k < 3; ++k) R.cc.xcost[k] = g_L.xc.c[k];
    R.cc.xparent = g_L.xc.parent;
    R.cc.nrow = E <= CONN_ROWS ? E : -1;
    R.cc.ok = 1;
  }
  __syncthreads();
  sc_copy_out(sb, par, &R.cc, sizeof(ScoutConn));
  sc_publish(C, par, tag, SC_CONN);
  CONNPROF_CONNECT(_c0, _c1, _c2);
}

__device__ void sc_end(const Ctx& C, int par, unsigned tag, int opt) {
  if (opt && uni(g_L.two_scouts)) {
    if (threadIdx.x == 0) g_L.sr.cc.ok = 0;
    __syncthreads();
    sc_copy_out(C.Q.scb, par, &g_L.sr.cc, sizeof(ScoutConn));
    sc_publish(C, par, tag, SC_CONN);
  } else {
    sc_publish(C, par, tag, SC_DONE);
  }
}

__device__ void scout_pre_connect(const Ctx& C, int par, int tb) {
  ScoutRec& R = g_L.sr;
  QState& S = g_L.S;
  if (threadIdx.x == 0) {
    ScoutPre& P = R.pre;
    for (int k = 0; k < 3; ++k) P.sol[k] = g_L.eg_cost[0][k] + g_L.xn.c[k];
    P.need = P.sol[0] < S.cbest[0];
    int flag = 0;
    if (P.need) {
      const int f = g_L.eg_first[0];
      if (f > S.n_pts) {
        flag = 1;
      } else {
        const int lv = f == 0 ? 0 : f - 1;
        if (lv != 0) {
          for (int j = 0; j < NJ; ++j) g_L.ext[j] = g_L.eg_start[0][j] + lv * g_L.eg_step[0][j];
          flag = 2;
        }
      }
    }
    P.flag = flag;
    P.nv = 0;
    P.ok = 1;
    P.sel.id = -1;
    P.sel.parent = -1;
    g_L.flag = flag;
    g_L.n_via = 0;
    g_L.nn_t = S.n[tb];
    g_L.cur = g_L.xc;
  }
  __syncthreads();
  const int flag = uni(g_L.flag);
  if (!flag) return;
  const int vcap = S.via_cap, st0 = S.status, ph0 = S.phase;
  __syncthreads();
  if (threadIdx.x == 0) S.via_cap = PRE_VIA;
  __syncthreads();
  via_chain(C, flag == 1 ? g_L.xn.q : g_L.ext);
  if (threadIdx.x == 0) {
    ScoutPre& P = R.pre;
    P.ok = S.status == st0;
    S.status = st0;
    S.phase = ph0;
    S.via_cap = vcap;
    P.nv = g_L.n_via;
    P.sel = g_L.sel;
    for (int j = 0; j < NJ; ++j) { P.sel_start[j] = g_L.sel_start[j]; P.sel_target[j] = g_L.sel_target[j]; }
    g_L.n_via = 0;
  }
  drain();
  __syncthreads();
  const int nw = uni(R.pre.ok ? R.pre.nv : 0) * (int)(sizeof(ViaNode) / 8);
  const unsigned long long* src = reinterpret_cast<const unsigned long long*>(C.Q.via);
  unsigned long long* dst = reinterpret_cast<unsigned long long*>(&C.Q.scb->pre_via[par][0]);
  for (int w = threadIdx.x; w < nw; w += BLOCK) st_agent(&dst[w], ld_agent(&src[w]));
}

__device__ void scout_pre_publish(const Ctx& C, int par, unsigned tag, bool valid) {
  const ScoutRec& R = g_L.sr;
  PreRec& P = g_L.prer;
  if (threadIdx.x == 0) {
    P.t = valid ? R.nn.t : -1;
    P.X = R.nn.X;
    P.nn_id = R.nn.id;
    P.nn_d = R.nn.d;
    P.first = R.e[0].first;
    for (int j = 0; j < NJ; ++j) {
      P.xr[j] = R.nn.q[j]; P.nn_q[j] = R.e[0].s[j]; P.ext[j] = R.ex.ext[j]; P.end[j] = R.ex.end[j];
      P.sel_q[j] = R.pre.sel.q[j]; P.sel_start[j] = R.pre.sel_start[j]; P.sel_target[j] = R.pre.sel_target[j];
    }
    for (int k = 0; k < 3; ++k) {
      P.nn_c[k] = R.nn.c[k]; P.acc[k] = R.ex.acc[k]; P.cn_c[k] = R.cn.c[k]; P.sol[k] = R.pre.sol[k];
      P.sel_c[k] = R.pre.sel.c[k];
    }
    P.cn_ok = R.cn.ok;
    P.cn_d = R.cn.d;
    P.cn_id = R.cn.id;
    P.XB = R.cn.X;
    P.cn_first = R.cn.e.first;
    P.pre_ok = R.cn.ok && R.pre.ok;
    P.flag = R.pre.flag;
// ... 20 lines not shown
    const unsigned long long sz = ld_agent(&C.Q.scb->cur_sz);
    const int n0 = (int)((sz >> 20) & 0xfffff), n1 = (int)(sz & 0xfffff);
    g_L.cnt = max(X, t == 0 ? n0 : n1);
    g_L.found = max(XB, t == 0 ? n1 : n0);
  }
  __syncthreads();
  const int Xn = uni(g_L.cnt), XBn = uni(g_L.found);
  __syncthreads();
  if (Xn <= X) return false;
  __builtin_amdgcn_fence(__ATOMIC_ACQUIRE, "agent");
  drain();
  __syncthreads();
  bool again = Xn - X > 64;
  if (!again) {
    double dp;
    tail_scan(C, t, g_L.xr, X, Xn, &dp);
    again = dp < R.nn.d;
  }
  if (!again) return false;
  if (threadIdx.x == 0) {
    S.n[t] = Xn;
    S.n[1 - t] = XBn;
    S.prof[P_SC_REDONE]++;
    R.cn.ok = 0;
    R.pre.ok = 0;
    R.nn.ok = 0; R.ex.ok = 0; R.nr.ok = 0; R.n_choose = 0; R.n_rewire = 0; R.cc.ok = 0; R.cc.nfirst = -1;
  }
  __syncthreads();
  return true;
}

__device__ void scout_iteration(const Ctx& C, long long it, int t, int X, int opt, unsigned ver, int XB) {
  QState& S = g_L.S;
  ScoutRec& R = g_L.sr;
  ScoutBoard* sb = C.Q.scb;
  JobBoard* jb = C.Q.jb;
  const int par = (int)(it & (SCOUT_SLOTS - 1));
  const unsigned tag = (unsigned)(it + 1);
  (void)jb;
  unsigned long long _ts = threadIdx.x == 0 ? wall_clock64() : 0;
  TR_PASS(it);
  TR();
  if (threadIdx.x == 0) {
    S.prof[P_SC_PASSES]++;
    S.n[t] = X;
    S.n[1 - t] = XB;
    R.cn.ok = 0;
    R.pre.ok = 0;
    R.nn.ok = 0; R.ex.ok = 0; R.nr.ok = 0; R.n_choose = 0; R.n_rewire = 0; R.cc.ok = 0; R.cc.nfirst = -1;
    g_L.conn_ov = 0;
  }
  unsigned long long v0 = 0;
  if (threadIdx.x < 2 * NJ) v0 = ld_agent(&C.Q.sampler_jb->ring[it % SMP_RING].g[threadIdx.x]);
  if (opt) sc_publish(C, par, tag, SC_STARTED);
  if (threadIdx.x < 64) {
    const JobBoard* lb = C.Q.sampler_jb;
    const unsigned want = ring_tag(it, ver);
    const unsigned long long t0 = wall_clock64();
    int ok = 0;
    for (bool first_round = true;; first_round = false) {
      unsigned long long v = v0;
      if (!first_round && threadIdx.x < 2 * NJ) v = ld_agent(&lb->ring[it % SMP_RING].g[threadIdx.x]);
      const bool cur = threadIdx.x >= 2 * NJ || (unsigned)(v >> 32) == want;
      if (__ballot(!cur) == 0) {
        const unsigned hi = (unsigned)odd_lane_of_pair((int)(unsigned)v);
        if (threadIdx.x < 2 * NJ && !(threadIdx.x & 1))
          g_L.xr[threadIdx.x >> 1] = __longlong_as_double((long long)(((unsigned long long)hi << 32) | (unsigned)v));
        ok = 1;
        break;
      }
      if (__builtin_amdgcn_readfirstlane((int)(wall_clock64() - t0 > 2000))) break;
      __builtin_amdgcn_s_sleep(2);
    }
    if (threadIdx.x == 0) g_L.flag = ok;
  }
  __syncthreads();
  SC_PHASE(0);
  TR();
  if (!uni(g_L.flag) && !opt) {
    scout_pre_publish(C, par, tag, false);
    return;
  }
  if (!uni(g_L.flag)) {
    sc_copy_out(sb, par, &R.nn, sizeof(ScoutNN));
    sc_copy_out(sb, par, &R.nr, sizeof(ScoutNear));
    sc_copy_out(sb, par, &R.cn, sizeof(ScoutConnect));
    sc_copy_out(sb, par, &R.pre, sizeof(ScoutPre));
    sc_copy_out(sb, par, &R.n_choose, 4 * sizeof(int));
    sc_end(C, par, tag, opt);
    return;
  }
  int rp = 0;
redo:
  if (opt && sc_moved(C)) return;
  int nid;
  [[clang::always_inline]] nid = nearest(C, t, g_L.xr);
  if (threadIdx.x < 64) {
    const int lane = threadIdx.x;
    if (lane == 0) load_node(C, t, nid, &g_L.nn);
    wave_sync();
    double nq[NJ], xe[NJ];
#pragma unroll
    for (int j = 0; j < NJ; ++j) { nq[j] = g_L.nn.q[j]; xe[j] = g_L.xr[j]; }
    double s = 0.0;
#pragma unroll
    for (int j = 0; j < NJ; ++j) { const double d = xe[j] - nq[j]; s += d * d; }
    const double d = sqrt(s);
    const double nn_l = g_L.nn.q[lane & 7];
    double x_l = g_L.xr[lane & 7];
    step_towards_w(rev_mask(&g_rb), nq, xe, S.step, lane, nn_l, x_l);
    if (lane < NJ) {
      R.nn.q[lane] = g_L.xr[lane];
      g_L.ext[lane] = x_l;
      g_L.eg_start[0][lane] = nn_l;
      g_L.eg_target[0][lane] = x_l;
    } else if (lane < NJ + 3) {
      const int k = lane - NJ;
      R.nn.c[k] = g_L.nn.c[k];
      g_L.eg_base[0][k] = g_L.nn.c[k];
    } else if (lane == NJ + 3) {
      R.nn.d = d < 10000.0 ? d : 10000.0;
      R.nn.id = nid; R.nn.X = X; R.nn.t = t; R.nn.ok = 1;
      g_L.eg_need[0] = 1;
    }
  }
  __syncthreads();
  if (opt) {
    sc_copy_out(sb, par, &R.nn, sizeof(ScoutNN));
    sc_publish(C, par, tag, SC_NN);
  }
  SC_PHASE(1);
  TR();
  if (opt && sc_moved(C)) return;
  edge_costs(C, 1);
  if (threadIdx.x == 0) {
    if (!opt) {
      for (int j = 0; j < NJ; ++j) { R.ex.ext[j] = g_L.eg_target[0][j]; R.ex.step[j] = g_L.eg_step[0][j]; R.ex.end[j] = g_L.eg_end[0][j]; }
      for (int k = 0; k < 3; ++k) R.ex.acc[k] = g_L.eg_acc[0][k];
    }
    R.ex.ok = 1;
  }
  if (threadIdx.x == 0) g_L.spec = OV_NONE;
  const bool spec_conn = !opt && !sc_stale(C, tag);
  int cid_s = 0;
  if (spec_conn) {
    const int tb = 1 - t;
    [[clang::always_inline]] cid_s = nearest(C, tb, g_L.eg_end[0]);
    if (threadIdx.x == 0) {
      load_node(C, tb, cid_s, &g_L.xc);
      for (int j = 0; j < NJ; ++j) { g_L.eg_start[1][j] = g_L.xc.q[j]; g_L.eg_target[1][j] = g_L.eg_end[0][j]; }
      for (int k = 0; k < 3; ++k) g_L.eg_base[1][k] = g_L.xc.c[k];
      g_L.eg_need[1] = 1;
    }
    for (int e = 2 + threadIdx.x; e < MAXE; e += BLOCK) g_L.eg_need[e] = 0;
    __syncthreads();
    edge_costs(C, 2);
    [[clang::always_inline]] edge_validity(C, 2, false, P_XEXPAND, OV_NONE, t);
  } else {
    CONNPROF_CLOCK(_e0);
    [[clang::always_inline]] edge_validity(C, 1, false, P_XEXPAND, opt ? OV_NEAR_EXPAND : OV_NONE, t, -1,
                                           opt ? EARLY_EXPAND : EARLY_NONE, par);
    CONNPROF_EXPAND(_e0, opt);
  }
  if (opt) sc_first_send(C, EARLY_EXPAND, par, 1);
  if (threadIdx.x == 0) {
    if (!opt) {
      for (int j = 0; j < NJ; ++j) { R.e[0].s[j] = g_L.eg_start[0][j]; R.e[0].g[j] = g_L.eg_target[0][j]; }
      for (int k = 0; k < 3; ++k) R.e[0].acc[k] = g_L.eg_acc[0][k];
      R.e[0].first = g_L.eg_first[0];
    }
    const int f = g_L.eg_first[0];
    g_L.ext_nn = f > S.n_pts;
    if (g_L.ext_nn) {
      for (int j = 0; j < NJ; ++j) g_L.xn.q[j] = g_L.eg_end[0][j];
      for (int k = 0; k < 3; ++k) g_L.xn.c[k] = g_L.eg_cost[0][k];
    } else {
      for (int j = 0; j < NJ; ++j) g_L.xn.q[j] = g_L.xr[j];
      g_L.xn.c[0] = 10000.0; g_L.xn.c[1] = 0.0; g_L.xn.c[2] = 0.0;
    }
    g_L.xn.id = X;
    g_L.xn.parent = g_L.nn.id;
    g_L.ext_bp = 0;
  }
  __syncthreads();
  if (!opt && (C.Q.pre_refresh & 1) && rp < 2 && pre_newer(C, t, X, XB)) {
    X = uni(g_L.cnt);
    XB = uni(g_L.found);
    rp++;
    goto redo;
  }
  if (spec_conn && uni(g_L.ext_nn)) {
    const int tb = 1 - t;
    const int cid = cid_s;
    if (threadIdx.x < NJ) {
      const int j = threadIdx.x;
      g_L.eg_start[0][j] = g_L.eg_start[1][j]; g_L.eg_target[0][j] = g_L.eg_target[1][j];
      g_L.eg_step[0][j] = g_L.eg_step[1][j]; g_L.eg_end[0][j] = g_L.eg_end[1][j];
    }
    if (threadIdx.x < 3) {
      const int k = threadIdx.x;
      g_L.eg_base[0][k] = g_L.eg_base[1][k]; g_L.eg_acc[0][k] = g_L.eg_acc[1][k]; g_L.eg_cost[0][k] = g_L.eg_cost[1][k];
    }
    if (threadIdx.x == 0) {
      g_L.eg_first[0] = g_L.eg_first[1];
      double s = 0.0;
      for (int j = 0; j < NJ; ++j) { double d = g_L.xn.q[j] - g_L.xc.q[j]; s += d * d; }
      const double d = sqrt(s);
      for (int j = 0; j < NJ; ++j) R.cn.q[j] = g_L.xn.q[j];
      R.cn.d = d < 10000.0 ? d : 10000.0;
      R.cn.id = cid; R.cn.X = XB; R.cn.t = tb;
    }
    __syncthreads();
    if (threadIdx.x == 0) {
      for (int j = 0; j < NJ; ++j) { R.cn.e.s[j] = g_L.eg_start[0][j]; R.cn.e.g[j] = g_L.eg_target[0][j]; }
      for (int k = 0; k < 3; ++k) { R.cn.e.acc[k] = g_L.eg_acc[0][k]; R.cn.c[k] = g_L.xc.c[k]; }
      R.cn.e.first = g_L.eg_first[0];
      R.cn.ok = 1;
    }
    __syncthreads();
    scout_pre_connect(C, par, tb);
  }
  if (!opt && (C.Q.pre_refresh & 2) && rp < 2 && pre_newer(C, t, X, XB)) {
    X = uni(g_L.cnt);
    XB = uni(g_L.found);
    rp++;
    goto redo;
  }
  if (!opt) {
    scout_pre_publish(C, par, tag, true);
    return;
  }
  if (uni(g_L.sc_stale_f)) {
    sc_copy_out(sb, par, &R.nr, sizeof(ScoutNear));
    sc_copy_out(sb, par, &R.n_choose, 4 * sizeof(int));
    sc_publish(C, par, tag, SC_DONE);
    return;
  }
  sc_publish(C, par, tag, SC_EXPAND);
  SC_PHASE(2);
  TR();
  if (sc_moved(C)) return;
  if (!(uni(g_L.ext_nn) && take_spec(OV_NEAR_EXPAND))) {
    CONNPROF_CLOCK(_n0);
    [[clang::always_inline]] near_set<20>(C, t, g_L.xn.q, X);
    CONNPROF_NEAR2(_n0);
  }
  if (threadIdx.x < 20) {
    R.nr.lo_i[threadIdx.x] = g_L.lo_i[threadIdx.x]; R.nr.lo_c[threadIdx.x] = g_L.lo_c[threadIdx.x];
    R.nr.hi_i[threadIdx.x] = g_L.hi_i[threadIdx.x]; R.nr.hi_c[threadIdx.x] = g_L.hi_c[threadIdx.x];
  }
  if (threadIdx.x == 0) {
    for (int j = 0; j < NJ; ++j) R.nr.q[j] = g_L.xn.q[j];
    R.nr.nk = g_L.nk; R.nr.n_lo = g_L.n_lo; R.nr.n_hi = g_L.n_hi;
    R.nr.X = X; R.nr.t = t; R.nr.ok = 1;
  }
  if (threadIdx.x < 64) {
    const int E = choose_prefix();
    if (threadIdx.x == 0) {
      g_L.cnt = E;
      g_L.found = -1;
      R.n_choose = E;
    }
  }
  __syncthreads();
  sc_copy_out(sb, par, &R.nr, sizeof(ScoutNear));
  const int E = uni(g_L.cnt);
  if (threadIdx.x < E) {
    const int e = threadIdx.x;
    NodeRef nd;
    load_node(C, t, g_L.lo_i[e], &nd);
    for (int j = 0; j < NJ; ++j) { g_L.eg_start[e][j] = nd.q[j]; g_L.eg_target[e][j] = g_L.xn.q[j]; }
    for (int k = 0; k < 3; ++k) g_L.eg_base[e][k] = nd.c[k];
    g_L.eg_near[e] = nd.id;
  } else if (threadIdx.x >= 64 && (int)threadIdx.x - 64 < min(g_L.n_hi, MAXE)) {
    const TreeDev& T = C.Q.tr[t];
    const int i = (int)threadIdx.x - 64;
    int v = g_L.hi_i[i];
    const int cap = g_L.S.cap;
    BCHK(v, cap, SMP_SITE, t);
    double q[NJ];
    for (int j = 0; j < NJ; ++j) q[j] = T.q[(size_t)j * cap + v];
    const double c0 = T.cost[v];
    const int pv = T.parent[v];
    for (int j = 0; j < NJ; ++j) g_L.sc_hq[i][j] = q[j];
    g_L.sc_hc[i] = c0;
    g_L.sc_hp[i] = pv;
  }
  sc_publish(C, par, tag, SC_NEAR);
  SC_PHASE(3);
  TR();
  if (sc_moved(C)) return;
  if (E > 0) {
    edge_costs(C, E);
    if (threadIdx.x < E) g_L.eg_need[threadIdx.x] = g_L.eg_cost[threadIdx.x][0] <= g_L.xn.c[0];
    for (int e = E + threadIdx.x; e < MAXE; e += BLOCK) g_L.eg_need[e] = 0;
    __syncthreads();
    [[clang::always_inline]] edge_validity(C, E, false, P_XCHOOSE, OV_NONE, 0, -1, EARLY_CHOOSE, par);
    sc_first_send(C, EARLY_CHOOSE, par, E);
    if (threadIdx.x < 64) {
      const bool fr = (int)threadIdx.x < E && g_L.eg_need[threadIdx.x] && g_L.eg_first[threadIdx.x] > S.n_pts;
      const unsigned long long fm = __ballot(fr);
      if (threadIdx.x == 0 && fm) g_L.found = (int)__builtin_ctzll(fm);
    }
    if (uni(g_L.sc_stale_f)) { sc_publish(C, par, tag, SC_DONE); return; }
  } else {
    sc_copy_out(sb, par, &R.n_choose, 4 * sizeof(int));
    if (sc_stale(C, tag)) { sc_publish(C, par, tag, SC_DONE); return; }
  }
  sc_publish(C, par, tag, SC_CHOOSE);
  SC_PHASE(4);
  TR();
  if (uni(g_L.found) >= 0) {
    if (threadIdx.x == 0) {
      g_L.n_via = 0;
      g_L.nn_t = X;
      load_node(C, t, g_L.eg_near[g_L.found], &g_L.cur);
    }
    __syncthreads();
    via_chain(C, g_L.xn.q);
    if (threadIdx.x == 0) {
      g_L.xn.id = g_L.sel.id;
      g_L.xn.parent = g_L.sel.parent;
      for (int j = 0; j < NJ; ++j) g_L.xn.q[j] = g_L.sel.q[j];
      for (int k = 0; k < 3; ++k) g_L.xn.c[k] = g_L.sel.c[k];
      g_L.ext_bp = 1;
      g_L.n_via = 0;
    }
    __syncthreads();
  }
  SC_PHASE(5);
  TR();
  if (!uni(g_L.ext_nn || g_L.ext_bp)) { sc_end(C, par, tag, opt); return; }
  if (sc_moved(C)) return;
  if (threadIdx.x < 64) {
    const int n = g_L.nk, lane = threadIdx.x;
    const int m = min(n >= S.max_near ? S.max_near : n, min(g_L.n_hi, MAXE));
    const bool ok = lane < m && g_L.xn.c[0] < g_L.sc_hc[g_L.n_hi - 1 - lane];
    const int c = __popcll(__ballot(ok));
    if (lane == 0) g_L.cnt = c;
  }
  __syncthreads();
  const int cnt = uni(g_L.cnt);
  if (cnt > 0) {
    if (threadIdx.x < cnt * NJ) {
      const int e = threadIdx.x / NJ, j = threadIdx.x - e * NJ;
      g_L.eg_start[e][j] = g_L.xn.q[j];
      g_L.eg_target[e][j] = g_L.sc_hq[g_L.n_hi - 1 - e][j];
    } else if (threadIdx.x >= 256 && threadIdx.x < 256 + cnt) {
      const int e = threadIdx.x - 256;
      for (int k = 0; k < 3; ++k) g_L.eg_base[e][k] = g_L.xn.c[k];
      g_L.eg_near[e] = g_L.hi_i[g_L.n_hi - 1 - e];
    }
    __syncthreads();
    edge_costs(C, cnt);
    if (threadIdx.x < cnt) {
      const int e = threadIdx.x, v = g_L.eg_near[e], h = g_L.n_hi - 1 - e;
      g_L.eg_need[e] = (v != g_L.xn.parent) && (g_L.sc_hp[h] != 0) && (g_L.eg_cost[e][0] < g_L.sc_hc[h]);
    }
    for (int e = cnt + threadIdx.x; e < MAXE; e += BLOCK) g_L.eg_need[e] = 0;
    if (threadIdx.x == 0) R.n_rewire = cnt;
    __syncthreads();
    CONNPROF_CLOCK(_r0);
    [[clang::always_inline]] edge_validity(C, cnt, false, P_XREWIRE, OV_NONE, 1 - t, -1, EARLY_REWIRE, par, true);
    CONNPROF_REWIRE(_r0);
    sc_first_send(C, EARLY_REWIRE, par, cnt);
  } else {
    sc_copy_out(sb, par, &R.n_choose, 4 * sizeof(int));
  }
  sc_publish(C, par, tag, SC_DONE);
  SC_PHASE(6);
  TR();
  if (sc_moved(C)) return;
  if (uni(g_L.two_scouts)) {
    [[clang::always_inline]] scout_connect(C, it, t, par, tag);
  }
  TR();
}
#undef SC_PHASE

__device__ __forceinline__ void scout_ctx(Ctx& C, int which) {
  C.Q.scb = C.Q.scbs[which];
  C.Q.sjb = C.Q.sjbs[which];
  C.Q.svia = C.Q.svias[which];
  C.Q.sworkers = C.Q.sworkers_s[which];
  C.Q.sampler_jb = C.Q.jb;
  C.Q.jb = C.Q.sjb;
  C.Q.nworkers = C.Q.sworkers;
  C.Q.via = C.Q.svia;
  C.Q.rows = nullptr;
  C.Q.trace = nullptr;
  C.Q.ttff = nullptr;
}

__device__ __noinline__ void scout_main(Ctx& C, int which) {
  {
    const int* src = reinterpret_cast<const int*>(C.Q.st);
    int* dst = reinterpret_cast<int*>(&g_L.S);
    for (int i = threadIdx.x; i < (int)(sizeof(QState) / sizeof(int)); i += BLOCK) dst[i] = src[i];
  }
  __syncthreads();
  if (threadIdx.x < 32) g_L.S.prof[threadIdx.x] = 0;
  if (threadIdx.x == 0) {
    g_L.count_slot = 0;
    g_L.job_seq = 0;
    g_L.in_job = 0;
    g_L.ov_local = 0; g_L.conn_ov = 0; g_L.conn_ov_n = 0;
    CONNPROF_RESET();
    g_L.n_via = 0;
    g_L.near_blo = ~0ull;
    g_L.near_bhi = 0;
    g_L.spec = OV_NONE;
    g_L.sp_on = 0;
    st_agent(&C.Q.scb->xcc, xcc_id() + 1);
    g_L.two_scouts = C.Q.nscouts >= 2;
    g_L.rec_grp = -1;
    TR_ROLE(which + 1 < 3 ? which + 1 : 3, -1, g_L.trole);
  }
  __syncthreads();
  unsigned last = 0;
  unsigned long long t_last = wall_clock64();
  const bool retired = which >= 2 && uni(g_L.S.tree_opt && g_L.S.have_sol);
  unsigned l_w0 = 0, l_ver = 0;
  int l_X = 0, l_XB = 0;
  if (threadIdx.x == 0) { g_L.sc_mod = 0; g_L.sc_t = 0; g_L.sc_rerun = 0; }
  for (int k = 0; !retired; k ^= 1) {
    if (threadIdx.x == 0) {
      int go = 0;
      if (ld_agent(&C.Q.scb->stop)) {
        go = -1;
      } else {
        const unsigned long long r0 = ld_agent(&C.Q.scb->req[0]), r1 = ld_agent(&C.Q.scb->req[1]);
        const unsigned long long r2 = ld_agent(&C.Q.scb->req[2]);
        const unsigned tag = (unsigned)(r0 >> 32);
        if (tag > last && (unsigned)(r1 >> 32) == tag && (unsigned)(r2 >> 32) == tag) {
          go = 1;
          g_L.cnt = (int)(unsigned)r0;
          g_L.nn_t = (int)(unsigned)r1;
          g_L.found = (int)(unsigned)r2;
          g_L.tree_expand = (int)tag;
        } else if (last && C.Q.early_ask && ((l_w0 >> 29) & 1u) &&
                   (ld_agent(&C.Q.scb->rwb[(l_w0 >> 28) & 1u]) & 0xfffu) != g_L.sc_mod &&
                   (long long)ld_agent(&C.Q.scb->cur) < (long long)last - 1) {
          go = 2;
        } else if (wall_clock64() - t_last > 200000000ull) {
          go = -1;
        }
      }
      g_L.sp_go[k] = go;
    }
    __syncthreads();
    const int go = uni(g_L.sp_go[k]);
    if (go < 0) break;
    if (go == 0) {
      __builtin_amdgcn_s_sleep(2);
      continue;
    }
    unsigned w0, ver, tag;
    int X, XB;
    if (go == 1) {
      const unsigned r1w = (unsigned)uni(g_L.nn_t);
      w0 = (unsigned)uni(g_L.cnt);
      ver = r1w & 0xfffffu;
      tag = (unsigned)uni(g_L.tree_expand);
      XB = uni(g_L.found);
      X = (int)(w0 & ((1u << 28) - 1));
      __syncthreads();
      if (threadIdx.x == 0) g_L.sc_mod = (r1w >> 20) & 0xfffu;
    } else {
      w0 = l_w0; ver = l_ver; tag = last; X = l_X; XB = l_XB;
    }
    const int t = (int)(w0 >> 28) & 1, opt = (int)(w0 >> 29) & 1;
    __syncthreads();
    if (go == 1 && !opt && C.Q.pre_delay > 0) {
      const long long k = (long long)tag - 1;
      for (int r = 0;; r ^= 1) {
        if (threadIdx.x == 0) {
          const long long cur = (long long)ld_agent(&C.Q.scb->cur);
          const int go = cur >= k - C.Q.pre_delay || ld_agent(&C.Q.scb->stop);
          if (go) {
            const unsigned long long sz = ld_agent(&C.Q.scb->cur_sz);
            const int n0 = (int)((sz >> 20) & 0xfffff), n1 = (int)(sz & 0xfffff);
            g_L.cnt = max(X, t == 0 ? n0 : n1);
            g_L.found = max(XB, t == 0 ? n1 : n0);
          }
          g_L.sp_go[r] = go;
        }
        __syncthreads();
        if (uni(g_L.sp_go[r])) break;
        __builtin_amdgcn_s_sleep(2);
      }
      X = uni(g_L.cnt);
      XB = uni(g_L.found);
      __syncthreads();
    }
    l_w0 = w0; l_ver = ver; l_X = X; l_XB = XB;
    const unsigned long long tb = wall_clock64();
    if (threadIdx.x == 0) g_L.S.prof[P_SC_IDLE] += tb - t_last;
    for (;;) {
      if (opt && C.Q.early_ask) {
        int st = 0;
        for (int r = 0;; r ^= 1) {
          if (threadIdx.x == 0) {
            const unsigned b = ld_agent(&C.Q.scb->rwb[t]);
            int v;
            if ((b & 0xfffu) == g_L.sc_mod) v = 1;
            else if (ld_agent(&C.Q.scb->stop) || (long long)ld_agent(&C.Q.scb->cur) > (long long)tag - 1) v = -1;
            else if (ld_agent(&C.Q.scb->rwe[t]) == b) { v = 1; g_L.sc_mod = b & 0xfffu; }
            else v = 0;
            g_L.rb_go[r] = v;
          }
          __syncthreads();
          st = uni(g_L.rb_go[r]);
          if (st != 0) break;
          __builtin_amdgcn_s_sleep(1);
        }
        __syncthreads();
        if (st < 0) break;
      }
      if (threadIdx.x == 0) { g_L.sc_t = t; g_L.sc_rerun = 0; g_L.sc_k = (long long)tag - 1; }
      __builtin_amdgcn_fence(__ATOMIC_ACQUIRE, "agent");
      drain();
      __syncthreads();
      [[clang::always_inline]] scout_iteration(C, (long long)tag - 1, t, X, opt, ver, XB);
      if (!opt || !uni(g_L.sc_rerun)) break;
      __syncthreads();
    }
    last = tag;
    t_last = wall_clock64();
    if (threadIdx.x == 0) g_L.S.prof[P_SC_BUSY] += t_last - tb;
  }
  if (threadIdx.x == 0) {
    st_agent(&C.Q.jb->stop, 1);
    for (int k = 0; k < 32; ++k) st_agent(&C.Q.scb->prof[k], g_L.S.prof[k]);
    st_agent(&C.Q.scb->conn_ov_n, (unsigned long long)g_L.conn_ov_n);
    CONNPROF_STORE(C);
  }
}

__device__ __forceinline__ void sampler_body(const Ctx& C, SamplerLds& L) {
  JobBoard* jb = C.Q.jb;
  {
    const int* src = reinterpret_cast<const int*>(C.Q.st);
    int* dst = reinterpret_cast<int*>(&L.S);
    for (int i = threadIdx.x; i < (int)(sizeof(QState) / sizeof(int)); i += BLOCK) dst[i] = src[i];
  }
  if (threadIdx.x == 0) { L.ver = 0; L.next = 0; }
  __syncthreads();
  unsigned long long t_last = wall_clock64();
  for (int k = 0;; k ^= 1) {
    if (threadIdx.x == 0) {
      int go = 0;
      if (ld_agent(&jb->stop)) {
        go = -1;
      } else {
        const int ver = ld_agent(&jb->s_ver);
        const long long cur = (long long)ld_agent(reinterpret_cast<const unsigned long long*>(&jb->s_iter));
        if (ver != L.ver) {
          L.S.have_sol = ld_agent(&jb->s_have_sol);
          for (int c = 0; c < 3; ++c) L.S.cbest[c] = __longlong_as_double((long long)ld_agent(&jb->s_cbest[c]));
          if (ld_agent(&jb->s_ver) == ver) { L.ver = ver; L.next = cur + 1; }
        }
        if (L.next < cur + 1) L.next = cur + 1;
        if (L.ver > 0 && ver == L.ver && L.next <= cur + SMP_RING - 1) go = 1;
        else if (wall_clock64() - t_last > 200000000ull) go = -1;
      }
      L.go[k] = go;
    }
    __syncthreads();
    const int go = uni(L.go[k]);
    if (go < 0) break;
    if (go == 0) {
      __builtin_amdgcn_s_sleep(2);
      continue;
    }
    const long long it = L.next;
    const int st = sample_conf(L.S, (uint32_t)it, L.W, L.out);
    ring_check_params(L, it);
    if (st == 0 && threadIdx.x < RING_G) {
      unsigned w;
      if (threadIdx.x < 2 * NJ) {
        const unsigned long long bits = (unsigned long long)__double_as_longlong(L.out[threadIdx.x >> 1]);
        w = (threadIdx.x & 1) ? (unsigned)(bits >> 32) : (unsigned)bits;
      } else {
        w = ring_param((int)threadIdx.x - 2 * NJ, L.S.have_sol, L.S.cbest);
      }
      st_agent(&jb->ring[it % SMP_RING].g[threadIdx.x], granule((int)ring_tag(it, L.ver), w));
    }
    if (threadIdx.x == 0) L.next = it + 1;
    t_last = wall_clock64();
    __syncthreads();
  }
}

__device__ __noinline__ void sampler_main(const Ctx& C, SamplerLds& L) { sampler_body(C, L); }


__global__ void __launch_bounds__(BLOCK) plan_kernel(const RobotDev* __restrict__ rb, SceneDev sc,
                                                     const MapCfg* __restrict__ mc, QueryDev* qs, int nq, int scout_base,
                                                     int helper_base, int iters) {
  const int b = (int)blockIdx.x;
  const int r8 = (nq + 7) / 8 * 8;
  const int so = b - scout_base, srole = scout_base > 0 && b >= scout_base && b < helper_base ? so / r8 : -1;
// ... 53 lines not shown
    g_L.sc_seen = 0;
    g_L.sc_dead = 0;
    for (int k = 0; k < SCOUT_SLOTS; ++k) { g_L.asked[k] = 0; g_L.asked_conn[k] = 0; g_L.asked_pre[k] = 0; }
    g_L.rec_grp = -1;
    g_L.count_slot = 0;
    g_L.job_seq = 0;
    g_L.in_job = 0;
    g_L.ov_local = 0;
    g_L.S = *C.Q.st;
    if (g_L.S.phase == 0 && g_L.S.t0 == 0) {
      g_L.S.t0 = wall_clock64();
      if (g_L.S.has_deadline) g_L.S.deadline = g_L.S.t0 + g_L.S.budget_ticks;
    }
    g_L.n_via = 0;
    g_L.near_blo = ~0ull;
    g_L.near_bhi = 0;
    g_L.smp_ver = 0;
    for (int s = 0; s < C.Q.nscouts && s < 2; ++s)
      for (int t = 0; t < 2; ++t) {
        st_agent(reinterpret_cast<int*>(&C.Q.scbs[s]->rwb[t]), g_L.S.rewires[t]);
        st_agent(reinterpret_cast<int*>(&C.Q.scbs[s]->rwe[t]), g_L.S.rewires[t]);
      }
    drain();
    TR_ROLE(0, 0, 0);
  }
  __syncthreads();
  TR();
  if (uni(g_L.S.status == 0 && g_L.S.phase == 0)) {
    if (threadIdx.x < 2 * NJ) {
      const int c = threadIdx.x / NJ, j = threadIdx.x - c * NJ;
      g_L.u.tile.tq[c][j] = c == 0 ? g_L.S.qs[j] : g_L.S.qg[j];
    }
    __syncthreads();
    collide_tile<PLAN_CT>((&g_rb), C.sc, (&g_mc), 2, g_L.u.tile.tq, g_L.S.self, g_L.S.map, g_L.u.tile.T);
    if (threadIdx.x == 0 && (g_L.u.tile.T.coll[0] || g_L.u.tile.T.coll[1])) {
      g_L.S.status = g_L.u.tile.T.coll[0] ? -2 : -3;
      g_L.S.phase = 2;
    }
    __syncthreads();
    TR();
  }
  if (uni(g_L.S.status == 0 && g_L.S.phase == 0) && threadIdx.x < 2) {
    const int t = threadIdx.x, cap = g_L.S.cap;
    const TreeDev& T = C.Q.tr[t];
    for (int j = 0; j < NJ; ++j) st_coord(T, cap, j, 0, t == 0 ? g_L.S.qs[j] : g_L.S.qg[j]);
    for (int k = 0; k < 3; ++k) T.cost[(size_t)k * cap] = 0.0;
    T.parent[0] = 0;
    T.first_child[0] = -1;
    T.next_sib[0] = -1;
    T.prev_sib[0] = -1;
  }
  __syncthreads();
  for (int it = threadIdx.x; it < 2 * PATCH_K * NJ; it += BLOCK) {
    const int t = it / (PATCH_K * NJ), r = it - t * (PATCH_K * NJ), k = r / NJ, j = r - k * NJ;
    const int i = g_L.S.n[t] - PATCH_K + k;
    if (i >= 0) g_L.pc_q[t][i & (PATCH_K - 1)][j] = C.Q.tr[t].q[(size_t)j * g_L.S.cap + i];
  }
  __syncthreads();
  if (uni(g_L.S.status == 0 && g_L.S.phase == 0 && C.Q.nscouts > 0 && C.Q.pre_commit && C.Q.sampler)) {
    drain();
    __syncthreads();
    if (threadIdx.x == 0) {
      sample_version(C);
      sample_publish(C, true);
      bool fenced = false;
      const long long j = g_L.S.iter;
      for (int ahead = 0; ahead < C.Q.nscouts; ++ahead)
        scout_ask(C, j + ahead, (ahead & 1) ? 1 - g_L.S.A : g_L.S.A, true, fenced);
    }
    __syncthreads();
  }
  if (uni(g_L.S.status == 0 && g_L.S.phase == 0)) {
    if (threadIdx.x == 0) {
      load_node(C, 1, 0, &g_L.xn);
      load_node(C, 0, 0, &g_L.xc);
    }
    __syncthreads();
    connect_graphs(C, 0);
    if (threadIdx.x == 0)
      g_L.S.phase = (g_L.S.have_sol || (g_L.S.max_checked && g_L.S.checked >= g_L.S.max_checked)) ? 2 : 1;
    __syncthreads();
  }
  const unsigned long long t_launch = wall_clock64();
  for (int k = 0; k < iters; ++k) {
    if (uni(g_L.S.status != 0 || g_L.S.phase != 1)) break;
    if (((C.Q.lquota > 0 || C.Q.lticks > 0) && (k & 7) == 7) || (C.Q.abort && (k & (ABORT_EVERY - 1)) == ABORT_EVERY - 1)) {
      if (threadIdx.x == 0)
        g_L.go_end = (C.Q.lquota > 0 && ld_agent(C.Q.lfin) >= (unsigned)C.Q.lquota) ||
                     (C.Q.lticks > 0 && (long long)(wall_clock64() - t_launch) > C.Q.lticks) ||
                     (C.Q.abort && __hip_atomic_load(C.Q.abort, __ATOMIC_RELAXED, __HIP_MEMORY_SCOPE_SYSTEM) != 0u);
      __syncthreads();
      if (uni(g_L.go_end)) break;
    }
    iteration(C);
  }
  if (threadIdx.x == 0) {
    if (C.Q.lquota > 0 && (g_L.S.phase == 2 || g_L.S.status != 0))
      __hip_atomic_fetch_add(C.Q.lfin, 1u, __ATOMIC_RELAXED, __HIP_MEMORY_SCOPE_AGENT);
    if (g_L.S.phase == 2 && g_L.S.t_end == 0) g_L.S.t_end = wall_clock64();
    JOBPROF_COLLECT(C);
    *C.Q.st = g_L.S;
    if (C.Q.jb) st_agent(&C.Q.jb->stop, 1);
    for (int s = 0; s < C.Q.nscouts; ++s) st_agent(&C.Q.scbs[s]->stop, 1);
  }
}

__global__ void __launch_bounds__(BLOCK) boards_reset_kernel(const QueryDev* qs, int ns) {
  const int per = 1 + 2 * ns, q = (int)blockIdx.x / per, w = (int)blockIdx.x - q * per;
  const QueryDev& Q = qs[q];
  char* base = w == 0 ? (char*)Q.jb : w <= ns ? (char*)Q.sjbs[w - 1] : (char*)Q.scbs[w - 1 - ns];
  const size_t bytes = w == 0 || w <= ns ? sizeof(JobBoard) : sizeof(ScoutBoard);
  uint4* p4 = reinterpret_cast<uint4*>(base);
  const size_t n4 = bytes / sizeof(uint4);
  for (size_t i = threadIdx.x; i < n4; i += BLOCK) p4[i] = make_uint4(0u, 0u, 0u, 0u);
  for (size_t i = n4 * sizeof(uint4) + threadIdx.x; i < bytes; i += BLOCK) base[i] = 0;
}

__global__ void path_kernel(QueryDev* qs, int* counts) {
  QueryDev Q = qs[blockIdx.x];
  if (threadIdx.x != 0) return;
  const QState& S = *Q.st;
  int cap = S.cap;
  int* ps = Q.path_nodes;
  int* pg = Q.path_nodes + cap;
  int ns = 0, ng = 0;
  if (S.have_sol) {
    int s_id = S.conn_start ? S.nB.id : S.nA.id, s_par = S.conn_start ? S.nB.parent : S.nA.parent;
    int g_id = S.conn_start ? S.nA.id : S.nB.id, g_par = S.conn_start ? S.nA.parent : S.nB.parent;
    while (s_id != 0 && ns < cap) { ps[ns++] = s_id; s_id = s_par; s_par = Q.tr[0].parent[s_id]; }
    while (g_id != 0 && ng < cap) { pg[ng++] = g_id; g_id = g_par; g_par = Q.tr[1].parent[g_id]; }
    for (int i = 0; i < ns / 2; ++i) { int t = ps[i]; ps[i] = ps[ns - 1 - i]; ps[ns - 1 - i] = t; }
  }
  counts[blockIdx.x * 2] = ns;
  counts[blockIdx.x * 2 + 1] = ng;
}


__global__ void path_edges_kernel(const QueryDev* qs, int q, int ns, int ng, double* out) {
  const QueryDev& Q = qs[q];
  const int cap = Q.st->cap;
  for (int k = blockIdx.x * blockDim.x + threadIdx.x; k < (ns + ng) * 2 * NJ; k += gridDim.x * blockDim.x) {
    const int e = k / (2 * NJ), w = k - e * (2 * NJ), j = w % NJ;
    const int t = e < ns ? 0 : 1;
    const int id = e < ns ? Q.path_nodes[e] : Q.path_nodes[cap + (e - ns)];
    const double* src = w < NJ ? Q.tr[t].e_start : Q.tr[t].e_target;
    out[k] = src[(size_t)j * cap + id];
  }
}

template <bool INL>
__device__ __forceinline__ void near_probe_body(const double* tqv, const double* tcost, int cap, int n,
                                                const double* queries, const int* excl, int m, double r, int reps, int* nn,
                                                int* nk, int* lo, int* hi, unsigned long long* ticks, const float* tqf) {
  Ctx C;
  C.Q.jb = nullptr;
  C.Q.scan_min = 0;
  C.Q.tr[0].q = const_cast<double*>(tqv);
  C.Q.tr[0].qf = const_cast<float*>(tqf);
  C.Q.tr[0].cost = const_cast<double*>(tcost);
  if (threadIdx.x == 0) {
    g_L.in_job = 0;
    g_L.ov_local = 0;
    g_L.S.n[0] = n;
    g_L.S.cap = cap;
    g_L.S.near_r = r;
    g_L.near_blo = ~0ull;
    g_L.near_bhi = 0;
// ... 137 lines not shown
```

### squirrel_motion_planner_amd/csrc/smp_plan.h

```cpp
#pragma once
#include <stddef.h>
#include <stdint.h>

#include "smp_types.h"

namespace smp {

constexpr int MAX_PTS = 32;
constexpr int MAX_NEAR = 32;
#ifndef SMP_MAXE
#define SMP_MAXE 24
#endif
constexpr int MAXE = SMP_MAXE;

struct NodeRef {
  double q[NJ];
  double c[3];
  int id;
  int parent;
};

struct TreeDev {
  double* q;
  double* cost;
  int* parent;
  int* first_child;
  int* next_sib;
  int* prev_sib;
  double* e_start;
  double* e_target;
  float* qf;
};

struct QState {
  int status;
  int phase;
  int A;
  int have_sol, conn_start;
  int n[2], edges[2], rewires[2];
  int cap, via_cap;
  long long iter, max_iter;
  long long max_checked;
  long long checked, valid, first_iter, last_iter;
  long long nn_nodes, near_nodes;
  long long smp_hits;
  long long sc_nn, sc_near, sc_edge_hit, sc_edge_miss;
  long long sc_conn_row, sc_conn_batch;
  unsigned long long sc_wait;
  unsigned long long prof[32];
  unsigned long long t0, t_first, t_end, deadline;
  unsigned long long budget_ticks;
  int has_deadline;
  int stop_margin;
  double cbest[3], h0[3];
  NodeRef nB, nA;
  double qs[NJ], qg[NJ];
  double Crev[36], Cpr[4], ctr_rev[6], ctr_pr[2];
  double env_x[2], env_y[2];
  double near_r, step, opt_thresh;
  int n_pts, max_near, tree_opt, informed, self, map;
  unsigned long long seed;
  unsigned query;
  long long n_rows;
};

struct ViaNode {
  double q[NJ];
  double c[3];
  double e_start[NJ];
  double e_target[NJ];
  int id, parent;
};

constexpr int TILE_CT_MAX = BLOCK / 64;
constexpr int JOB_SLOTS = MAXE * (MAX_PTS + 1);
constexpr int JOB_TILES = 256;
static_assert(JOB_TILES * TILE_CT_MAX >= JOB_SLOTS, "a job of 8-configuration tiles fits the result granules");
__host__ __device__ inline int job_tile_ct(int slots, int W, int fixed) {
  if (fixed > 0) return (slots + fixed - 1) / fixed <= JOB_TILES ? fixed : TILE_CT_MAX;
  const int helpers = W - 1 < JOB_TILES ? W - 1 : JOB_TILES;
  for (int ct = 1; ct < TILE_CT_MAX; ct <<= 1)
    if ((slots + ct - 1) / ct <= helpers) return ct;
  return TILE_CT_MAX;
}
constexpr int JOB_WORDS = 1 + 4 * NJ * MAXE;
constexpr int SMP_RING = 16;
constexpr int SCAN_P = 64;
constexpr int SCAN_PNEAR = 32;
constexpr int SCAN_W = 2 + 2 * 3 * MAX_NEAR;
constexpr int SCAN_WORDS = 33;
__host__ __device__ inline unsigned ring_tag(long long it, unsigned ver) {
  return ((unsigned)it & 0xffffffu) << 8 | (ver & 0xffu);
}
constexpr int RING_PARAMS = 5;
constexpr int RING_G = 2 * NJ + RING_PARAMS;
__device__ inline unsigned ring_param(int k, int have_sol, const double* cbest) {
  if (k == 0) return (unsigned)have_sol;
  const unsigned long long b = (unsigned long long)__double_as_longlong(cbest[1 + ((k - 1) >> 1)]);
  return ((k - 1) & 1) ? (unsigned)(b >> 32) : (unsigned)b;
}
struct JobBoard {
  int stop;
  int pad0[7];
  unsigned long long dbg[12];
  unsigned long long pay[JOB_WORDS];
  int pad1[32 - (2 * JOB_WORDS) % 32];
  unsigned long long res[JOB_TILES];
  int pad2[32 - (2 * JOB_TILES) % 32];
  unsigned long long spay[64];
  int s_ver, s_have_sol;
  long long s_iter;
  unsigned long long s_cbest[3];
  int pad6[22];
  struct {
    unsigned long long g[RING_G];
  } ring[SMP_RING];
  unsigned long long sres[SCAN_P][SCAN_W];
};

constexpr int SCOUT_EDGES = 1 + 2 * MAX_NEAR;
constexpr int SCOUT_CHOOSE0 = 1, SCOUT_REWIRE0 = 1 + MAX_NEAR;
enum { SC_STARTED = 0, SC_NN = 1, SC_EXPAND = 2, SC_NEAR = 3, SC_CHOOSE = 4, SC_DONE = 5, SC_CONN = 6 };
struct ScoutNN {
  double q[NJ];
  double d;
  double c[3];
  int id, X, t, ok;
};
struct ScoutNear {
  double q[NJ];
// ... 1 lines not shown
  int lo_i[MAX_NEAR], hi_i[MAX_NEAR];
  double lo_c[MAX_NEAR], hi_c[MAX_NEAR];
};
struct ScoutEdge {
  double s[NJ], g[NJ];
  double acc[3];
  int first, pad;
};
static_assert(offsetof(ScoutEdge, first) % 8 == 0 && sizeof(ScoutEdge) - offsetof(ScoutEdge, first) == 8,
              "ScoutEdge: {first, pad} is the last 8-byte word");
struct ScoutExpand {
  double ext[NJ];
  double step[NJ], end[NJ];
  double acc[3];
  int ok, pad;
};
struct ScoutConnect {
  double q[NJ];
  double d;
  double c[3];
  int id, X, t, ok;
  ScoutEdge e;
};
constexpr int PRE_VIA = 16;
struct ScoutPre {
  int ok;
  int flag;
  int nv, need;
  double sol[3];
  NodeRef sel;
  double sel_start[NJ], sel_target[NJ];
};
constexpr int CONN_ROWS = 20;
static_assert(CONN_ROWS % 2 == 0 && CONN_ROWS <= MAXE, "ScoutConn: 8-byte words; the rows fill an edge batch");
struct ScoutConn {
  double q[NJ];
  double d;
  int id, X, t, excl;
  int nk, n_lo, n_hi, ok;
  int lo_i[MAX_NEAR], hi_i[MAX_NEAR];
  double lo_c[MAX_NEAR], hi_c[MAX_NEAR];
  double acc0[3];
  double pad0;
  double acc[MAX_NEAR][3];
  int first0, nfirst;
  int first[MAX_NEAR];
  double xq[NJ], xcost[3];
  int xparent, nrow;
  double rq[CONN_ROWS][NJ], rcost[CONN_ROWS][3];
  int rparent[CONN_ROWS];
};
struct PreRec {
  double xr[NJ];
  double nn_q[NJ];
  double nn_c[3];
  double nn_d;
  double ext[NJ], end[NJ];
  double acc[3];
  double cn_d, cn_c[3];
  double sol[3];
  double sel_q[NJ], sel_c[3];
  double sel_start[NJ], sel_target[NJ];
  int nn_id, X, t, first;
  int cn_id, XB, cn_ok, cn_first;
  int pre_ok, flag, nv, need;
  int sel_id, sel_parent, pad[2];
};
constexpr int PRE_GRANULES = (int)(sizeof(PreRec) / 4);
static_assert(sizeof(PreRec) % 8 == 0 && PRE_GRANULES <= 4 * 64, "pre-solution record: one granule per lane of 4 waves");

struct ScoutRec {
  ScoutNN nn;
  ScoutExpand ex;
  ScoutConnect cn;
  ScoutPre pre;
  ScoutNear nr;
  ScoutConn cc;
  int n_choose, n_rewire, pad[2];
  ScoutEdge e[SCOUT_EDGES];
};
constexpr int MAX_SCOUTS = 8;
constexpr int SCOUT_SLOTS = 16;
static_assert(SCOUT_SLOTS > MAX_SCOUTS && (SCOUT_SLOTS & (SCOUT_SLOTS - 1)) == 0, "record slots");
struct ScoutBoard {
  unsigned long long req[3];
  int stop;
  int xcc;
  unsigned rwb[2], rwe[2];
  int pad0[4];
  unsigned long long cur;
  unsigned long long cur_sz;
  int pad2[28];
  unsigned long long stage[SCOUT_SLOTS];
  unsigned long long cgo;
  unsigned long long conn_ov_n;
  unsigned long long cprof[6];
  unsigned long long prof[32];
  ScoutRec rec[SCOUT_SLOTS];
  ViaNode pre_via[SCOUT_SLOTS][PRE_VIA];
  unsigned long long pre_g[SCOUT_SLOTS][PRE_GRANULES];
};

constexpr int ABORT_EVERY = 64;
struct QueryDev {
  QState* st;
  JobBoard* jb;
  JobBoard* sampler_jb;
  int nscouts;
  int pre_delay;
  int pre_commit;
  int early_ask;
  int conn_check;
  int pre_refresh;
  ScoutBoard* scbs[MAX_SCOUTS];
  JobBoard* sjbs[MAX_SCOUTS];
  ViaNode* svias[MAX_SCOUTS];
  int sworkers_s[MAX_SCOUTS];
  ScoutBoard* scb;
  JobBoard* sjb;
  ViaNode* svia;
  int sworkers;
  int* trace;
  unsigned* lfin;
  int lquota;
  long long lticks;
  unsigned* ttff;
  const unsigned* abort;
  int scan_min;
  int scan_pnn, scan_pnear;
  int scan_nshift;
  int scan_ps0;
  int nworkers;
  int tile_ct;
  int sampler;
  TreeDev tr[2];
  ViaNode* via;
  int* stack;
  double* rows;
  long long rows_cap;
  int* path_nodes;
  int conn_ov_max;
};

}
```

Measured before the change: 5.167 million.

## Tag scout record words so consumers validate sections without stage-word handshakes

Scout records are now stored as tagged 32-bit granules: every word carries an iteration/build tag. The consumer loads all pending sections at once and accepts each stage whose words all carry the expected tag, instead of first polling a stage word and then copying the whole record. This aims to cut the producer-consumer latency and the extra copy pass between scout and planner blocks. In exchange it doubles the bytes written per payload, adds build counters and per-wave ballot masks, and caps iterations per launch so the tag bits cannot overflow.

```diff
diff --git a/include/smp_gpu.h b/include/smp_gpu.h
--- a/include/smp_gpu.h
+++ b/include/smp_gpu.h
@@ -89,6 +89,8 @@
   int64_t scout_conn_row_hits;
   int64_t scout_conn_batch_hits;
   int64_t scout_conn_ov_hits;
+  int64_t scout_stages_taken;
+  int64_t scout_stage_rounds;
 } smp_stats;
 
 typedef struct smp_result {
diff --git a/squirrel_motion_planner_amd/_lib.py b/squirrel_motion_planner_amd/_lib.py
--- a/squirrel_motion_planner_amd/_lib.py
+++ b/squirrel_motion_planner_amd/_lib.py
@@ -55,7 +55,8 @@
                 ("scout_near_hits", _i64), ("scout_edge_hits", _i64), ("scout_edge_misses", _i64),
                 ("scout_wait_seconds", _d), ("scout_phase_seconds", _d * 32), ("helpers", ctypes.c_int32),
                 ("scout", ctypes.c_int32), ("time_first_solution_host", _d), ("scout_conn_row_hits", _i64),
-                ("scout_conn_batch_hits", _i64), ("scout_conn_ov_hits", _i64)]
+                ("scout_conn_batch_hits", _i64), ("scout_conn_ov_hits", _i64),
+                ("scout_stages_taken", _i64), ("scout_stage_rounds", _i64)]
 
 
 class Result(ctypes.Structure):
diff --git a/squirrel_motion_planner_amd/csrc/smp_api_plan.cpp b/squirrel_motion_planner_amd/csrc/smp_api_plan.cpp
--- a/squirrel_motion_planner_amd/csrc/smp_api_plan.cpp
+++ b/squirrel_motion_planner_amd/csrc/smp_api_plan.cpp
@@ -541,6 +541,8 @@
     st.scout_conn_row_hits = s.sc_conn_row;
     st.scout_conn_batch_hits = s.sc_conn_batch;
     st.scout_conn_ov_hits = (int64_t)c.scout_conn_ov[i];
+    st.scout_stages_taken = s.sc_stages;
+    st.scout_stage_rounds = s.sc_rounds;
     st.scout_wait_seconds = (double)s.sc_wait / p->wall_rate_hz;
     for (int k = 0; k < 32; ++k) {
       const bool count = k == 8 || k == 11 || (k >= 20 && k < 28) || k == 30;
diff --git a/squirrel_motion_planner_amd/csrc/smp_kernels.hip b/squirrel_motion_planner_amd/csrc/smp_kernels.hip
--- a/squirrel_motion_planner_amd/csrc/smp_kernels.hip
+++ b/squirrel_motion_planner_amd/csrc/smp_kernels.hip
@@ -377,6 +377,9 @@
   int tbar;
 #endif
   int sp_on, sp_stage, sp_go[2];
+  int sp_bld, sp_new[2], sp_st;
+  unsigned sp_wave[2][BLOCK / 64];
+  unsigned sc_build;
   double fnn_d;
   int fnn_id;
 #ifdef SMP_SCAN_PROF
@@ -529,7 +532,7 @@
   S.edges[t]++;
 }
 
-__device__ bool spec_stage(const Ctx& C, int s, unsigned long long wait = 0);
+__device__ bool spec_stage(const Ctx& C, int s, unsigned long long wait = 0, int lim = -1, bool once = false);
 __device__ __forceinline__ int scan_parts(const Ctx& C, int near, int nodes) {
   int P = min(min(C.Q.nworkers, SCAN_P), near ? min(min(C.Q.scan_pnear, SCAN_PNEAR), max(8, nodes >> C.Q.scan_nshift)) : C.Q.scan_pnn);
   if (g_L.in_job) P = min(P, max(C.Q.nworkers - g_L.u.job.ntiles, 8));
@@ -2112,41 +2115,45 @@
 __device__ __forceinline__ int sc_stale_now(const ScoutBoard* sb) {
   return (long long)ld_agent(&sb->cur) > g_L.sc_k || ld_agent(&sb->stop);
 }
+__device__ __forceinline__ unsigned sc_gtag() { return sg_tag(g_L.sc_k, g_L.sc_build); }
 __device__ __forceinline__ void sc_early_send(const Ctx& C, int early, int epar, int E, bool read_stale) {
   if (early == EARLY_NONE) return;
   ScoutBoard* sb = C.Q.scb;
-  ScoutRec* rec = &sb->rec[epar];
+  unsigned long long* g = sb->g[epar];
+  const unsigned gt = sc_gtag();
   if (read_stale && threadIdx.x == 0) g_L.sc_stale_f = sc_stale_now(sb);
   const int g0 = early == EARLY_EXPAND ? 0 : early == EARLY_CHOOSE ? SCOUT_CHOOSE0 : SCOUT_REWIRE0;
-  for (int i = threadIdx.x; i < E * EDGE_EARLY_W; i += BLOCK) {
-    const int e = i / EDGE_EARLY_W, k = i - e * EDGE_EARLY_W;
+  if (early != EARLY_EXPAND) E = min(E, SCOUT_CAND);
+  for (int i = threadIdx.x; i < E * 2 * EDGE_EARLY_W; i += BLOCK) {
+    const int e = i / (2 * EDGE_EARLY_W), h = i - e * (2 * EDGE_EARLY_W), k = h >> 1;
     const double v = k < NJ ? g_L.eg_start[e][k] : k < 2 * NJ ? g_L.eg_target[e][k - NJ] : g_L.eg_acc[e][k - 2 * NJ];
-    st_agent(reinterpret_cast<unsigned long long*>(&rec->e[g0 + e]) + k, (unsigned long long)__double_as_longlong(v));
+    const unsigned long long b = (unsigned long long)__double_as_longlong(v);
+    st_agent(&g[sg_of(offsetof(ScoutRec, e)) + (g0 + e) * (EDGE_G + 1) + h], granule((int)gt, (unsigned)(b >> (32 * (h & 1)))));
   }
   if (early == EARLY_EXPAND) {
     constexpr int XW = (int)(sizeof(ScoutExpand) / 8);
     static_assert(XW == 3 * NJ + 3 + 1 && offsetof(ScoutExpand, ok) == (XW - 1) * 8, "ScoutExpand: ext, step, end, acc, {ok, pad}");
-    const int k = (int)threadIdx.x - 64;
-    if (k >= 0 && k < XW) {
+    const int h = (int)threadIdx.x - 64;
+    if (h >= 0 && h < 2 * XW) {
+      const int k = h >> 1;
       unsigned long long w;
       if (k == XW - 1) w = *reinterpret_cast<const unsigned long long*>(&g_L.sr.ex.ok);
       else w = (unsigned long long)__double_as_longlong(k < NJ ? g_L.eg_target[0][k] : k < 2 * NJ ? g_L.eg_step[0][k - NJ] :
                                                         k < 3 * NJ ? g_L.eg_end[0][k - 2 * NJ] : g_L.eg_acc[0][k - 3 * NJ]);
-      st_agent(reinterpret_cast<unsigned long long*>(&rec->ex) + k, w);
-    }
-  } else {
-    const int k = (int)threadIdx.x - (BLOCK - 64);
-    if (k >= 0 && k < 2) st_agent(reinterpret_cast<unsigned long long*>(&rec->n_choose) + k,
-                                  reinterpret_cast<const unsigned long long*>(&g_L.sr.n_choose)[k]);
+      st_agent(&g[sg_of(offsetof(ScoutRec, ex)) + h], granule((int)gt, (unsigned)(w >> (32 * (h & 1)))));
+    }
+  } else if (threadIdx.x == BLOCK - 64) {
+    st_agent(&g[sg_header(early == EARLY_CHOOSE ? SC_CHOOSE : SC_DONE)], granule((int)gt, (unsigned)E));
   }
 }
 __device__ __forceinline__ void sc_first_send(const Ctx& C, int early, int epar, int E) {
   const int g0 = early == EARLY_EXPAND ? 0 : early == EARLY_CHOOSE ? SCOUT_CHOOSE0 : SCOUT_REWIRE0;
+  if (early != EARLY_EXPAND) E = min(E, SCOUT_CAND);
   if ((int)threadIdx.x < E) {
     const int e = threadIdx.x;
     const int first = g_L.eg_need[e] ? g_L.eg_first[e] : -1;
-    st_agent(reinterpret_cast<unsigned long long*>(&C.Q.scb->rec[epar].e[g0 + e]) + EDGE_EARLY_W,
-             (unsigned long long)(unsigned)first);
+    st_agent(&C.Q.scb->g[epar][sg_of(offsetof(ScoutRec, e)) + (g0 + e) * (EDGE_G + 1) + 2 * EDGE_EARLY_W],
+             granule((int)sc_gtag(), (unsigned)first));
   }
 }
 
@@ -2760,22 +2767,18 @@
   }
 }
 
-__device__ __forceinline__ void sc_copy_out(ScoutBoard* sb, int par, const void* p, int nbytes) {
-  const size_t off = (const char*)p - (const char*)&g_L.sr;
-  const unsigned long long* src = (const unsigned long long*)p;
-  unsigned long long* dst = (unsigned long long*)((char*)&sb->rec[par] + off);
-  for (int w = threadIdx.x; w < nbytes / 8; w += BLOCK) st_agent(&dst[w], src[w]);
-}
-__device__ __forceinline__ void sc_copy_in(const ScoutBoard* sb, int par, void* p, int nbytes) {
-  const size_t off = (const char*)p - (const char*)&g_L.sr;
-  unsigned long long* dst = (unsigned long long*)p;
-  const unsigned long long* src = (const unsigned long long*)((const char*)&sb->rec[par] + off);
-  for (int w = threadIdx.x; w < nbytes / 8; w += BLOCK) dst[w] = ld_agent(&src[w]);
+__device__ __forceinline__ void sc_send(ScoutBoard* sb, int par, const void* p, int nbytes) {
+  const unsigned gt = sc_gtag();
+  const unsigned* src = (const unsigned*)p;
+  unsigned long long* dst = &sb->g[par][((const char*)p - (const char*)&g_L.sr) / 4];
+  for (int w = threadIdx.x; w < nbytes / 4; w += BLOCK) st_agent(&dst[w], granule((int)gt, src[w]));
+}
+__device__ __forceinline__ void sc_send_count(ScoutBoard* sb, int par, int stage, int n) {
+  st_agent(&sb->g[par][stage == SC_CHOOSE ? sg_header(SC_CHOOSE) : sg_header(SC_DONE)], granule((int)sc_gtag(), (unsigned)n));
 }
 static_assert(sizeof(ScoutNN) % 8 == 0 && sizeof(ScoutNear) % 8 == 0 && sizeof(ScoutEdge) % 8 == 0 &&
               sizeof(ScoutExpand) % 8 == 0 && offsetof(ScoutRec, ex) % 8 == 0 && offsetof(ScoutRec, nr) % 8 == 0 &&
-              sizeof(ScoutConnect) % 8 == 0 && offsetof(ScoutRec, cn) % 8 == 0 && sizeof(ScoutConn) % 8 == 0 &&
-              sizeof(ScoutPre) % 8 == 0 && offsetof(ScoutRec, pre) % 8 == 0 && sizeof(ViaNode) % 8 == 0 &&
+              sizeof(ScoutConn) % 8 == 0 && sizeof(ViaNode) % 8 == 0 &&
               offsetof(ScoutRec, cc) % 8 == 0 && offsetof(ScoutRec, n_choose) % 8 == 0 && offsetof(ScoutRec, e) % 8 == 0,
               "scout record sections are 8-byte words");
 
@@ -2784,89 +2787,147 @@
 #define SMP_CONN_WAIT 2000
 #endif
 
-__device__ void spec_copy(const ScoutBoard* sb, int par, int have, int st);
-__device__ bool spec_stage(const Ctx& C, int s, unsigned long long wait) {
+template <int ST>
+__device__ __forceinline__ void sg_load(const unsigned long long* g, bool on, unsigned long long (&v)[SG_ROUND],
+                                        unsigned long long& h) {
+  constexpr int N = sg_count(ST);
+  if (!on) return;
+  if constexpr (sg_header(ST) >= 0) h = ld_agent(&g[sg_header(ST)]);
+#pragma unroll
+  for (int u = 0; u < SG_ROUND; ++u) {
+    const int i = (int)threadIdx.x + u * BLOCK;
+    if (u * BLOCK < N && i < N) v[u] = ld_agent(&g[sg_index(ST, i)]);
+  }
+}
+template <int ST>
+__device__ __forceinline__ bool sg_check(bool on, unsigned want, const unsigned long long (&v)[SG_ROUND],
+                                         unsigned long long h, int& need) {
+  constexpr int N = sg_count(ST);
+  need = 0;
+  if (!on) return false;
+  if constexpr (sg_header(ST) >= 0) {
+    if ((unsigned)(h >> 32) != want || (unsigned)h > (unsigned)SCOUT_CAND) return false;
+    need = (int)(unsigned)h * EDGE_G;
+  } else {
+    need = N;
+  }
+  bool ok = true;
+#pragma unroll
+  for (int u = 0; u < SG_ROUND; ++u) {
+    const int i = (int)threadIdx.x + u * BLOCK;
+    if (u * BLOCK < N && i < need && (unsigned)(v[u] >> 32) != want) ok = false;
+  }
+  return ok;
+}
+template <int ST>
+__device__ __forceinline__ void sg_store(const unsigned long long (&v)[SG_ROUND], unsigned long long h, int need) {
+  constexpr int N = sg_count(ST);
+  unsigned* dst = reinterpret_cast<unsigned*>(&g_L.sr);
+  if constexpr (sg_header(ST) >= 0) {
+    if (threadIdx.x == 0) dst[sg_header(ST)] = (unsigned)h;
+  }
+#pragma unroll
+  for (int u = 0; u < SG_ROUND; ++u) {
+    const int i = (int)threadIdx.x + u * BLOCK;
+    if (u * BLOCK < N && i < need) dst[sg_index(ST, i)] = (unsigned)v[u];
+  }
+}
+
+__device__ bool spec_stage(const Ctx& C, int s, unsigned long long wait, int lim, bool once) {
   if (!uni(g_L.sp_on)) return false;
   if (wait == 0) wait = SCOUT_WAIT;
-  const int have = uni(g_L.sp_stage);
+  int have = uni(g_L.sp_stage);
   if (have >= s) return true;
-  const ScoutBoard* sb = C.Q.scbs[uni(g_L.asked[g_L.S.iter & (SCOUT_SLOTS - 1)]) - 1];
+  if (lim < s) lim = s == SC_NN ? SC_EXPAND : s;
   const int par = (int)(g_L.S.iter & (SCOUT_SLOTS - 1));
-  const unsigned tag = (unsigned)(g_L.S.iter + 1);
+  const ScoutBoard* sb = C.Q.scbs[uni(g_L.asked[par]) - 1];
+  const unsigned long long* g = sb->g[par];
+  const unsigned stag = (unsigned)(g_L.S.iter + 1);
   const unsigned long long t0 = threadIdx.x == 0 ? wall_clock64() : 0;
   TR();
-  int got;
+  bool ok_s = false;
   for (int k = 0;; k ^= 1) {
+    const int bld = uni(g_L.sp_bld);
+    const unsigned want = sg_tag(g_L.S.iter, (unsigned)bld);
+    const bool o1 = have < SC_NN && lim >= SC_NN, o2 = have < SC_EXPAND && lim >= SC_EXPAND;
+    const bool o3 = have < SC_NEAR && lim >= SC_NEAR, o4 = have < SC_CHOOSE && lim >= SC_CHOOSE;
+    const bool o5 = have < SC_DONE && lim >= SC_DONE, o6 = have < SC_CONN && lim >= SC_CONN;
+    unsigned long long v1[SG_ROUND], v2[SG_ROUND], v3[SG_ROUND], v4[SG_ROUND], v5[SG_ROUND], v6[SG_ROUND];
+    unsigned long long h4 = 0, h5 = 0, hx = 0, sw = 0;
+    if (threadIdx.x == 0) sw = ld_agent(&sb->stage[par]);
+    sg_load<SC_NN>(g, o1, v1, hx);
+    sg_load<SC_EXPAND>(g, o2, v2, hx);
+    sg_load<SC_NEAR>(g, o3, v3, hx);
+    sg_load<SC_CHOOSE>(g, o4, v4, h4);
+    sg_load<SC_DONE>(g, o5, v5, h5);
+    sg_load<SC_CONN>(g, o6, v6, hx);
     if (threadIdx.x == 0) {
-      const unsigned long long v = ld_agent(&sb->stage[par]);
-      const unsigned lo = (unsigned)v;
+      const unsigned lo = (unsigned)sw;
+      const int sent = (int)(lo & 0xffu), build = (int)((lo >> 20) & 0xffu);
       const bool cur = ((lo >> 8) & 0xfffu) == (g_L.rw_at0 & 0xfffu);
-      int go = 0;
-      if ((unsigned)(v >> 32) != tag) go = -1;
-      else if (cur && (int)(lo & 0xffu) >= s) go = 1 + (int)(lo & 0xffu);
-      else if (wall_clock64() - t0 > wait) go = -1;
+      const bool late = once || wall_clock64() - t0 > wait;
+      int go;
+      if ((unsigned)(sw >> 32) != stag) go = once ? 0 : -1;
+      else if (!cur) go = late ? (once ? 0 : -1) : 0;
+      else if (build != bld) {
+        if (have >= SC_NN || late) go = once ? 0 : -1;
+        else { go = 3; g_L.sp_new[k] = build; }
+      }
+      else if ((lo & SG_END) && sent < s) go = once ? 1 : -1;
+      else go = late ? 2 : 1;
       g_L.sp_go[k] = go;
-    }
-    __syncthreads();
-    got = uni(g_L.sp_go[k]);
-    if (got != 0) break;
+      g_L.S.sc_rounds++;
+    }
+    int n1, n2, n3, n4, n5, n6;
+    const bool k1 = sg_check<SC_NN>(o1, want, v1, hx, n1), k2 = sg_check<SC_EXPAND>(o2, want, v2, hx, n2);
+    const bool k3 = sg_check<SC_NEAR>(o3, want, v3, hx, n3), k4 = sg_check<SC_CHOOSE>(o4, want, v4, h4, n4);
+    const bool k5 = sg_check<SC_DONE>(o5, want, v5, h5, n5), k6 = sg_check<SC_CONN>(o6, want, v6, hx, n6);
+    const unsigned wm = (o1 && __ballot(!k1) == 0 ? 1u << SC_NN : 0u) | (o2 && __ballot(!k2) == 0 ? 1u << SC_EXPAND : 0u) |
+                        (o3 && __ballot(!k3) == 0 ? 1u << SC_NEAR : 0u) | (o4 && __ballot(!k4) == 0 ? 1u << SC_CHOOSE : 0u) |
+                        (o5 && __ballot(!k5) == 0 ? 1u << SC_DONE : 0u) | (o6 && __ballot(!k6) == 0 ? 1u << SC_CONN : 0u);
+    if (lane_id() == 0) g_L.sp_wave[k][wave_id()] = wm;
+    __syncthreads();
+    const int go = uni(g_L.sp_go[k]);
+    if (go == 3) {
+      if (threadIdx.x == 0) g_L.sp_bld = g_L.sp_new[k];
+      __syncthreads();
+      if (once) return false;
+      continue;
+    }
+    int np = have;
+    if (go > 0) {
+      unsigned m = ~0u;
+#pragma unroll
+      for (int w = 0; w < BLOCK / 64; ++w) m &= g_L.sp_wave[k][w];
+      m = (unsigned)uni((int)m);
+      for (int x = max(have, (int)SC_STARTED) + 1; x <= lim && ((m >> x) & 1u); ++x) np = x;
+    }
+    ok_s = np >= s;
+    if (np > have) {
+      TR();
+      if (o1 && np >= SC_NN) sg_store<SC_NN>(v1, hx, n1);
+      if (o2 && np >= SC_EXPAND) sg_store<SC_EXPAND>(v2, hx, n2);
+      if (o3 && np >= SC_NEAR) sg_store<SC_NEAR>(v3, hx, n3);
+      if (o4 && np >= SC_CHOOSE) sg_store<SC_CHOOSE>(v4, h4, n4);
+      if (o5 && np >= SC_DONE) sg_store<SC_DONE>(v5, h5, n5);
+      if (o6 && np >= SC_CONN) sg_store<SC_CONN>(v6, hx, n6);
+      if (threadIdx.x == 0) {
+        g_L.sp_stage = np;
+        g_L.S.sc_stages += np - max(have, (int)SC_STARTED);
+      }
+      have = np;
+    }
+    if (ok_s || go < 0 || go == 2 || once) break;
     __builtin_amdgcn_s_sleep(1);
   }
-  if (threadIdx.x == 0) g_L.S.sc_wait += wall_clock64() - t0;
-  WAIT_CLOCK(s, t0);
+  if (threadIdx.x == 0 && !once) {
+    g_L.S.sc_wait += wall_clock64() - t0;
+    if (!ok_s) g_L.sp_on = 0;
+  }
+  if (!once) { WAIT_CLOCK(s, t0); }
+  __syncthreads();
   TR();
-  if (got < 0) {
-    if (threadIdx.x == 0) g_L.sp_on = 0;
-    __syncthreads();
-    return false;
-  }
-  spec_copy(sb, par, have, got - 1);
-  TR();
-  return true;
-}
-
-__device__ void spec_copy(const ScoutBoard* sb, int par, int have, int st) {
-  ScoutRec& R = g_L.sr;
-  const bool opt_now = uni(g_L.S.tree_opt && g_L.S.have_sol) != 0;
-  int off[8], nw[8], ns = 0;
-  auto add = [&](const void* p, int nbytes) {
-    off[ns] = (int)((const char*)p - (const char*)&R) / 8;
-    nw[ns] = nbytes / 8;
-    ++ns;
-  };
-  if (have < SC_NN && st >= SC_NN) add(&R.nn, sizeof(ScoutNN));
-  if (have < SC_EXPAND && st >= SC_EXPAND) { add(&R.e[0], sizeof(ScoutEdge)); add(&R.ex, sizeof(ScoutExpand)); }
-  if (have < SC_NEAR && st >= SC_NEAR) add(&R.nr, sizeof(ScoutNear));
-  if ((have < SC_CHOOSE && st >= SC_CHOOSE) || (have < SC_DONE && st >= SC_DONE)) add(&R.n_choose, 4 * sizeof(int));
-  if (opt_now && have < SC_CHOOSE && st >= SC_CHOOSE) add(&R.e[SCOUT_CHOOSE0], MAX_NEAR * sizeof(ScoutEdge));
-  if (opt_now && have < SC_DONE && st >= SC_DONE) add(&R.e[SCOUT_REWIRE0], MAX_NEAR * sizeof(ScoutEdge));
-  if (!opt_now && have < SC_DONE && st >= SC_DONE) { add(&R.cn, sizeof(ScoutConnect)); add(&R.pre, sizeof(ScoutPre)); }
-  if (have < SC_CONN && st >= SC_CONN) add(&R.cc, sizeof(ScoutConn));
-  int total = 0;
-  for (int i = 0; i < ns; ++i) total += nw[i];
-  const unsigned long long* src = reinterpret_cast<const unsigned long long*>(&sb->rec[par]);
-  unsigned long long* dst = reinterpret_cast<unsigned long long*>(&R);
-  constexpr int U = 4;
-  static_assert(sizeof(ScoutRec) / 8 <= U * BLOCK, "one round per record copy");
-  int idx[U];
-  unsigned long long v[U];
-#pragma unroll
-  for (int u = 0; u < U; ++u) {
-    const int w = (int)threadIdx.x + u * BLOCK;
-    idx[u] = -1;
-    if (w < total) {
-      int rem = w, i = 0;
-      while (rem >= nw[i]) { rem -= nw[i]; ++i; }
-      idx[u] = off[i] + rem;
-      v[u] = ld_agent(&src[idx[u]]);
-    }
-  }
-#pragma unroll
-  for (int u = 0; u < U; ++u)
-    if (idx[u] >= 0) dst[idx[u]] = v[u];
-  __syncthreads();
-  if (threadIdx.x == 0) g_L.sp_stage = st;
-  __syncthreads();
+  return ok_s;
 }
 
 __device__ void scout_ask(const Ctx& C, long long k, int tree, bool pre, bool& fenced, int x_snap = -1) {
@@ -3683,14 +3744,19 @@
   bool pre_ok = true;
   if (prerec) pre_ok = pre_read_round(sb, par, (unsigned)(S.iter + 1));
   if (threadIdx.x == 64) {
-    int st = -1;
+    int st = -1, st_e = -1, bld = -1;
     if (pre && !prerec) {
       const unsigned long long v = ld_agent(&sb->stage[par]);
       const unsigned lo = (unsigned)v;
-      if ((unsigned)(v >> 32) == (unsigned)(S.iter + 1) && ((lo >> 8) & 0xfffu) == (g_L.rw_at0 & 0xfffu))
+      if ((unsigned)(v >> 32) == (unsigned)(S.iter + 1) && ((lo >> 8) & 0xfffu) == (g_L.rw_at0 & 0xfffu)) {
         st = (int)(lo & 0xffu);
+        st_e = (lo & SG_END) ? max(st, (int)SC_DONE) : st;
+        bld = (int)((lo >> 20) & 0xffu);
+      }
     }
     g_L.sp_go[0] = st;
+    g_L.sp_st = st_e;
+    g_L.sp_bld = bld;
   }
   if (C.Q.sampler && threadIdx.x < 64) {
     JobBoard* jb = C.Q.jb;
@@ -3723,12 +3789,12 @@
     TR();
   } else if (threadIdx.x == 64 && C.Q.nscouts > 0) {
     scout_asks(C, 1 - g_L.S.A);
-    scout_ask_early(C, g_L.sp_go[0]);
+    scout_ask_early(C, g_L.sp_st);
   }
   TR();
   const int st = uni(g_L.sp_go[0]);
   __syncthreads();
-  if (pre && !prerec && st >= 0) spec_copy(sb, par, -1, st);
+  if (pre && !prerec && st >= SC_NN) spec_stage(C, SC_NN, 0, st, true);
   if (prer_ok && !uni(g_L.smp_hit) && uni(g_L.prer.t >= 0)) {
     if (threadIdx.x < NJ) g_L.xr[threadIdx.x] = g_L.prer.xr[threadIdx.x];
     if (threadIdx.x == 0) g_L.smp_hit = 1;
@@ -4592,12 +4658,11 @@
   TR_BARRIERS();
 }
 
-__device__ void sc_publish(const Ctx& C, int par, unsigned tag, int stage) {
+__device__ void sc_publish(const Ctx& C, int par, unsigned tag, int stage, bool end = false) {
   const unsigned long long t0 = threadIdx.x == 0 ? wall_clock64() : 0;
-  drain();
   __syncthreads();
   if (threadIdx.x == 0) {
-    st_agent(&C.Q.scb->stage[par], granule(tag, (unsigned)stage | (g_L.sc_mod & 0xfffu) << 8));
+    st_agent(&C.Q.scb->stage[par], granule(tag, sg_stage_word(stage, g_L.sc_mod, g_L.sc_build, end)));
     g_L.S.prof[P_SC_PUBLISH] += wall_clock64() - t0;
   }
   __syncthreads();
@@ -4711,20 +4776,13 @@
     R.cc.ok = 1;
   }
   __syncthreads();
-  sc_copy_out(sb, par, &R.cc, sizeof(ScoutConn));
-  sc_publish(C, par, tag, SC_CONN);
+  sc_send(sb, par, &R.cc, sizeof(ScoutConn));
+  sc_publish(C, par, tag, SC_CONN, true);
   CONNPROF_CONNECT(_c0, _c1, _c2);
 }
 
-__device__ void sc_end(const Ctx& C, int par, unsigned tag, int opt) {
-  if (opt && uni(g_L.two_scouts)) {
-    if (threadIdx.x == 0) g_L.sr.cc.ok = 0;
-    __syncthreads();
-    sc_copy_out(C.Q.scb, par, &g_L.sr.cc, sizeof(ScoutConn));
-    sc_publish(C, par, tag, SC_CONN);
-  } else {
-    sc_publish(C, par, tag, SC_DONE);
-  }
+__device__ void sc_end(const Ctx& C, int par, unsigned tag, int sent) {
+  sc_publish(C, par, tag, sent, true);
 }
 
 __device__ void scout_pre_connect(const Ctx& C, int par, int tb) {
@@ -4911,12 +4969,8 @@
     return;
   }
   if (!uni(g_L.flag)) {
-    sc_copy_out(sb, par, &R.nn, sizeof(ScoutNN));
-    sc_copy_out(sb, par, &R.nr, sizeof(ScoutNear));
-    sc_copy_out(sb, par, &R.cn, sizeof(ScoutConnect));
-    sc_copy_out(sb, par, &R.pre, sizeof(ScoutPre));
-    sc_copy_out(sb, par, &R.n_choose, 4 * sizeof(int));
-    sc_end(C, par, tag, opt);
+    sc_send(sb, par, &R.nn, sizeof(ScoutNN));
+    sc_end(C, par, tag, SC_NN);
     return;
   }
   int rp = 0;
@@ -4955,7 +5009,7 @@
   }
   __syncthreads();
   if (opt) {
-    sc_copy_out(sb, par, &R.nn, sizeof(ScoutNN));
+    sc_send(sb, par, &R.nn, sizeof(ScoutNN));
     sc_publish(C, par, tag, SC_NN);
   }
   SC_PHASE(1);
@@ -5060,9 +5114,7 @@
     return;
   }
   if (uni(g_L.sc_stale_f)) {
-    sc_copy_out(sb, par, &R.nr, sizeof(ScoutNear));
-    sc_copy_out(sb, par, &R.n_choose, 4 * sizeof(int));
-    sc_publish(C, par, tag, SC_DONE);
+    sc_end(C, par, tag, SC_EXPAND);
     return;
   }
   sc_publish(C, par, tag, SC_EXPAND);
@@ -5092,7 +5144,7 @@
     }
   }
   __syncthreads();
-  sc_copy_out(sb, par, &R.nr, sizeof(ScoutNear));
+  sc_send(sb, par, &R.nr, sizeof(ScoutNear));
   const int E = uni(g_L.cnt);
   if (threadIdx.x < E) {
     const int e = threadIdx.x;
@@ -5131,10 +5183,10 @@
       const unsigned long long fm = __ballot(fr);
       if (threadIdx.x == 0 && fm) g_L.found = (int)__builtin_ctzll(fm);
     }
-    if (uni(g_L.sc_stale_f)) { sc_publish(C, par, tag, SC_DONE); return; }
+    if (uni(g_L.sc_stale_f)) { sc_end(C, par, tag, SC_CHOOSE); return; }
   } else {
-    sc_copy_out(sb, par, &R.n_choose, 4 * sizeof(int));
-    if (sc_stale(C, tag)) { sc_publish(C, par, tag, SC_DONE); return; }
+    if (threadIdx.x == 0) sc_send_count(sb, par, SC_CHOOSE, 0);
+    if (sc_stale(C, tag)) { sc_end(C, par, tag, SC_CHOOSE); return; }
   }
   sc_publish(C, par, tag, SC_CHOOSE);
   SC_PHASE(4);
@@ -5159,7 +5211,11 @@
   }
   SC_PHASE(5);
   TR();
-  if (!uni(g_L.ext_nn || g_L.ext_bp)) { sc_end(C, par, tag, opt); return; }
+  if (!uni(g_L.ext_nn || g_L.ext_bp)) {
+    if (threadIdx.x == 0) sc_send_count(sb, par, SC_DONE, 0);
+    sc_end(C, par, tag, SC_DONE);
+    return;
+  }
   if (sc_moved(C)) return;
   if (threadIdx.x < 64) {
     const int n = g_L.nk, lane = threadIdx.x;
@@ -5194,9 +5250,9 @@
     CONNPROF_REWIRE(_r0);
     sc_first_send(C, EARLY_REWIRE, par, cnt);
   } else {
-    sc_copy_out(sb, par, &R.n_choose, 4 * sizeof(int));
-  }
-  sc_publish(C, par, tag, SC_DONE);
+    if (threadIdx.x == 0) sc_send_count(sb, par, SC_DONE, 0);
+  }
+  sc_publish(C, par, tag, SC_DONE, !uni(g_L.two_scouts));
   SC_PHASE(6);
   TR();
   if (sc_moved(C)) return;
@@ -5251,7 +5307,7 @@
   const bool retired = which >= 2 && uni(g_L.S.tree_opt && g_L.S.have_sol);
   unsigned l_w0 = 0, l_ver = 0;
   int l_X = 0, l_XB = 0;
-  if (threadIdx.x == 0) { g_L.sc_mod = 0; g_L.sc_t = 0; g_L.sc_rerun = 0; }
+  if (threadIdx.x == 0) { g_L.sc_mod = 0; g_L.sc_t = 0; g_L.sc_rerun = 0; g_L.sc_build = 0; }
   for (int k = 0; !retired; k ^= 1) {
     if (threadIdx.x == 0) {
       int go = 0;
@@ -5346,7 +5402,7 @@
         __syncthreads();
         if (st < 0) break;
       }
-      if (threadIdx.x == 0) { g_L.sc_t = t; g_L.sc_rerun = 0; g_L.sc_k = (long long)tag - 1; }
+      if (threadIdx.x == 0) { g_L.sc_t = t; g_L.sc_rerun = 0; g_L.sc_k = (long long)tag - 1; g_L.sc_build++; }
       __builtin_amdgcn_fence(__ATOMIC_ACQUIRE, "agent");
       drain();
       __syncthreads();
@@ -5566,7 +5622,7 @@
     __syncthreads();
   }
   const unsigned long long t_launch = wall_clock64();
-  for (int k = 0; k < iters; ++k) {
+  for (int k = 0; k < min(iters, LAUNCH_ITERS_MAX); ++k) {
     if (uni(g_L.S.status != 0 || g_L.S.phase != 1)) break;
     if (((C.Q.lquota > 0 || C.Q.lticks > 0) && (k & 7) == 7) || (C.Q.abort && (k & (ABORT_EVERY - 1)) == ABORT_EVERY - 1)) {
       if (threadIdx.x == 0)
diff --git a/squirrel_motion_planner_amd/csrc/smp_plan.h b/squirrel_motion_planner_amd/csrc/smp_plan.h
--- a/squirrel_motion_planner_amd/csrc/smp_plan.h
+++ b/squirrel_motion_planner_amd/csrc/smp_plan.h
@@ -46,6 +46,7 @@
   long long smp_hits;
   long long sc_nn, sc_near, sc_edge_hit, sc_edge_miss;
   long long sc_conn_row, sc_conn_batch;
+  long long sc_stages, sc_rounds;
   unsigned long long sc_wait;
   unsigned long long prof[32];
   unsigned long long t0, t_first, t_end, deadline;
@@ -213,6 +214,59 @@
 constexpr int MAX_SCOUTS = 8;
 constexpr int SCOUT_SLOTS = 16;
 static_assert(SCOUT_SLOTS > MAX_SCOUTS && (SCOUT_SLOTS & (SCOUT_SLOTS - 1)) == 0, "record slots");
+constexpr int SREC_G = (int)(sizeof(ScoutRec) / 4);
+constexpr int EDGE_G = (int)(sizeof(ScoutEdge) / 4) - 1;
+constexpr int SCOUT_CAND = 20;
+static_assert(SCOUT_CAND <= MAX_NEAR && SCOUT_CAND <= MAXE, "a section's candidates fit the record and an edge batch");
+static_assert(offsetof(ScoutEdge, pad) == sizeof(ScoutEdge) - 4, "ScoutEdge: the pad is the last 32-bit word");
+constexpr int sg_of(size_t byte_offset) { return (int)(byte_offset / 4); }
+constexpr int sg_count(int st) {
+  return st == SC_NN ? (int)(sizeof(ScoutNN) / 4)
+       : st == SC_EXPAND ? EDGE_G + (int)(sizeof(ScoutExpand) / 4)
+       : st == SC_NEAR ? (int)(sizeof(ScoutNear) / 4)
+       : st == SC_CHOOSE || st == SC_DONE ? SCOUT_CAND * EDGE_G
+       : st == SC_CONN ? (int)(sizeof(ScoutConn) / 4) : 0;
+}
+constexpr int sg_edge0(int st) { return st == SC_CHOOSE ? SCOUT_CHOOSE0 : st == SC_DONE ? SCOUT_REWIRE0 : 0; }
+__host__ __device__ constexpr int sg_index(int st, int i) {
+  return st == SC_NN ? sg_of(offsetof(ScoutRec, nn)) + i
+       : st == SC_EXPAND ? (i < EDGE_G ? sg_of(offsetof(ScoutRec, e)) + i : sg_of(offsetof(ScoutRec, ex)) + (i - EDGE_G))
+       : st == SC_NEAR ? sg_of(offsetof(ScoutRec, nr)) + i
+       : st == SC_CONN ? sg_of(offsetof(ScoutRec, cc)) + i
+       : sg_of(offsetof(ScoutRec, e)) + (sg_edge0(st) + i / EDGE_G) * (EDGE_G + 1) + i % EDGE_G;
+}
+constexpr int sg_header(int st) {
+  return st == SC_CHOOSE ? sg_of(offsetof(ScoutRec, n_choose)) : st == SC_DONE ? sg_of(offsetof(ScoutRec, n_rewire)) : -1;
+}
+constexpr int SG_ROUND = 2;
+constexpr bool sg_fit() {
+  for (int st = SC_NN; st <= SC_CONN; ++st)
+    if (sg_count(st) <= 0 || sg_count(st) > SG_ROUND * BLOCK) return false;
+  return true;
+}
+static_assert(sg_fit(), "every tagged section is read in one round of SG_ROUND loads per thread");
+constexpr bool sg_disjoint() {
+  bool used[SREC_G] = {};
+  for (int st = SC_NN; st <= SC_CONN; ++st) {
+    for (int i = -1; i < sg_count(st); ++i) {
+      const int g = i < 0 ? sg_header(st) : sg_index(st, i);
+      if (i < 0 && g < 0) continue;
+      if (g < 0 || g >= SREC_G || used[g]) return false;
+      used[g] = true;
+    }
+  }
+  return true;
+}
+static_assert(sg_disjoint(), "tagged sections: no word belongs to two of them");
+constexpr int LAUNCH_ITERS_MAX = 1 << 13;
+__host__ __device__ constexpr unsigned sg_tag(long long it, unsigned build) {
+  return (((unsigned)((unsigned long long)it / SCOUT_SLOTS)) & 0xffffffu) << 8 | (build & 0xffu);
+}
+static_assert(2 * MAX_NEAR < (1 << 8) && LAUNCH_ITERS_MAX < (1 << 24), "sg_tag: builds of an iteration, iterations of a launch");
+constexpr unsigned SG_END = 1u << 28;
+__host__ __device__ constexpr unsigned sg_stage_word(int stage, unsigned mod, unsigned build, bool end) {
+  return (unsigned)stage | (mod & 0xfffu) << 8 | (build & 0xffu) << 20 | (end ? SG_END : 0u);
+}
 struct ScoutBoard {
   unsigned long long req[3];
   int stop;
@@ -227,7 +281,7 @@
   unsigned long long conn_ov_n;
   unsigned long long cprof[6];
   unsigned long long prof[32];
-  ScoutRec rec[SCOUT_SLOTS];
+  unsigned long long g[SCOUT_SLOTS][SREC_G];
   ViaNode pre_via[SCOUT_SLOTS][PRE_VIA];
   unsigned long long pre_g[SCOUT_SLOTS][PRE_GRANULES];
 };
```

Result: no change. 5.206 million (median of 6 runs) (+0.8%).
